# cvlab-kaist/CoPoNeRF

Hardware: AMD Instinct MI355X
Metric: rendered rays/sec (RealEstate10K-shaped 256x256 stereo pair, full-image render, 64 samples/ray) (higher is better)
Workload: dtype f16 (fp16-input/fp32-accumulate MFMA for the per-sample MLPs; f32 decoder; f64 geometry island); 1 GPU; configs[1]: 256x256 stereo pair (narrow rig), full-image render 65536 rays x 64 samples, 1 pair(s) per GPU, render path only (z/rel_pose/flow given, val=True); chunk_rays=65536, lanes=1, pairs_per_gpu=1

## Files before the change

### coponerf_amd/csrc/ufc_conv4d.hip

```cpp
#include <algorithm>
#include <cstdlib>

#include "common.h"
#include "conv4d_geometry.h"

namespace {

__device__ __forceinline__ void gn_publish(double s1, double s2, double* __restrict__ stats, int b) {
    __shared__ int last_flag;
    __shared__ double tree[2][256];
    const unsigned W = gridDim.x * gridDim.y, me = blockIdx.x + gridDim.x * blockIdx.y, B = gridDim.z;
    unsigned long long* part = reinterpret_cast<unsigned long long*>(stats + 3 * (size_t)B + 2 * ((size_t)b * W));
    if (threadIdx.x == 0) {
        const unsigned long long o1 = __hip_atomic_exchange(part + 2 * me, (unsigned long long)__double_as_longlong(s1),
                                                            __ATOMIC_RELAXED, __HIP_MEMORY_SCOPE_AGENT);
        const unsigned long long o2 = __hip_atomic_exchange(part + 2 * me + 1, (unsigned long long)__double_as_longlong(s2),
                                                            __ATOMIC_RELAXED, __HIP_MEMORY_SCOPE_AGENT);
        unsigned zero;
        asm volatile("v_and_b32 %0, 0, %1\n\tv_and_b32 %0, %0, %2" : "=&v"(zero) : "v"((unsigned)o1), "v"((unsigned)o2));
        unsigned long long* cnt = reinterpret_cast<unsigned long long*>(stats + 2 * (size_t)B + b);
        const unsigned long long ticket = __hip_atomic_fetch_add(cnt, 1ULL + zero, __ATOMIC_RELAXED, __HIP_MEMORY_SCOPE_AGENT);
        last_flag = ticket == (unsigned long long)W - 1;
    }
    __syncthreads();
    if (!last_flag) return;
    double a1 = 0.0, a2 = 0.0;
    for (unsigned w = threadIdx.x; w < W; w += 256) {
        a1 += __longlong_as_double((long long)__hip_atomic_load(part + 2 * w, __ATOMIC_RELAXED, __HIP_MEMORY_SCOPE_AGENT));
        a2 += __longlong_as_double((long long)__hip_atomic_load(part + 2 * w + 1, __ATOMIC_RELAXED, __HIP_MEMORY_SCOPE_AGENT));
    }
    tree[0][threadIdx.x] = a1;
    tree[1][threadIdx.x] = a2;
    __syncthreads();
    for (int n = 128; n > 0; n >>= 1) {
        if ((int)threadIdx.x < n) {
            tree[0][threadIdx.x] += tree[0][threadIdx.x + n];
            tree[1][threadIdx.x] += tree[1][threadIdx.x + n];
        }
        __syncthreads();
    }
    if (threadIdx.x == 0) {
        stats[2 * (size_t)b] = tree[0][0];
        stats[2 * (size_t)b + 1] = tree[1][0];
    }
}

__device__ __forceinline__ void gn_publish_block(double s1, double s2, double* __restrict__ stats, int b) {
#pragma unroll
    for (int off = 32; off > 0; off >>= 1) {
        s1 += __shfl_xor(s1, off);
        s2 += __shfl_xor(s2, off);
    }
    __shared__ double red[8];
    const int lane = threadIdx.x & 63, wave = threadIdx.x >> 6;
    if (lane == 0) { red[wave * 2] = s1; red[wave * 2 + 1] = s2; }
    __syncthreads();
    gn_publish(red[0] + red[2] + red[4] + red[6], red[1] + red[3] + red[5] + red[7], stats, b);
}

__global__ __launch_bounds__(256) void conv4d_kernel(const float* __restrict__ x, const float* __restrict__ wq,
                                                     const float* __restrict__ bq, const float* __restrict__ ws,
                                                     const float* __restrict__ bs, int Cin, int Hq, int Wq, int Hs,
                                                     int Ws, int k, int s, int p, int Oq, int Pq_, int Os, int Ps_,
                                                     float* __restrict__ y, double* __restrict__ stats) {
    const int o = blockIdx.y, b = blockIdx.z, Cout = gridDim.y;
    const long long npos = (long long)Oq * Pq_ * Os * Ps_;
    const long long pos = (long long)blockIdx.x * blockDim.x + threadIdx.x;
    float val = 0.0f;
    const bool active = pos < npos;
    if (active) {
        int sx = (int)(pos % Ps_);
        long long t = pos / Ps_;
        const int sy = (int)(t % Os); t /= Os;
        const int qx = (int)(t % Pq_);
        const int qy = (int)(t / Pq_);
        const size_t cstride = (size_t)Hq * Wq * Hs * Ws;
        const float* xb = x + (size_t)b * Cin * cstride;
        float acc = bq[o] + bs[o];
        for (int c = 0; c < Cin; ++c) {
            const float* xc = xb + c * cstride;
            const float* wqc = wq + ((size_t)o * Cin + c) * k * k;
            const float* wsc = ws + ((size_t)o * Cin + c) * k * k;
            for (int i = 0; i < k; ++i)
                for (int j = 0; j < k; ++j) {
                    const int Y = qy * s + i - p, X = qx * s + j - p;
                    if (Y >= 0 && Y < Hq && X >= 0 && X < Wq) {
                        const float* base = xc + ((size_t)Y * Wq + X) * Hs * Ws;
                        float m = -INFINITY;
                        for (int dy = 0; dy < s; ++dy)
                            for (int dx = 0; dx < s; ++dx) {
                                const int yy = sy * s + dy, xx = sx * s + dx;
                                if (yy < Hs && xx < Ws) m = fmaxf(m, base[(size_t)yy * Ws + xx]);
                            }
                        acc += wqc[i * k + j] * m;
                    }
                    const int U = sy * s + i - p, Vv = sx * s + j - p;
                    if (U >= 0 && U < Hs && Vv >= 0 && Vv < Ws) {
                        float m = -INFINITY;
                        for (int dy = 0; dy < s; ++dy)
                            for (int dx = 0; dx < s; ++dx) {
                                const int yy = qy * s + dy, xx = qx * s + dx;
                                if (yy < Hq && xx < Wq) m = fmaxf(m, xc[(((size_t)yy * Wq + xx) * Hs + U) * Ws + Vv]);
                            }
                        acc += wsc[i * k + j] * m;
                    }
                }
        }
        val = acc;
        y[((size_t)b * Cout + o) * npos + pos] = acc;
    }
    double s1 = active ? (double)val : 0.0, s2 = active ? (double)val * val : 0.0;
    gn_publish_block(s1, s2, stats, b);
}

__global__ __launch_bounds__(256) void pool_support_kernel(const float* __restrict__ x, int Hs, int Ws, int s, int Os,
                                                           int Ps_, long long planes, float* __restrict__ out) {
    const long long total = planes * Os * Ps_;
    for (long long i = (long long)blockIdx.x * blockDim.x + threadIdx.x; i < total; i += (long long)gridDim.x * blockDim.x) {
        const int sx = (int)(i % Ps_);
        long long t = i / Ps_;
        const int sy = (int)(t % Os);
        const long long pl = t / Os;
        const float* base = x + pl * Hs * Ws;
        float m = -INFINITY;
        for (int dy = 0; dy < s; ++dy)
            for (int dx = 0; dx < s; ++dx) {
                const int yy = sy * s + dy, xx = sx * s + dx;
                if (yy < Hs && xx < Ws) m = fmaxf(m, base[(size_t)yy * Ws + xx]);
            }
        out[i] = m;
    }
}

__global__ __launch_bounds__(256) void pool_query_kernel(const float* __restrict__ x, int Hq, int Wq, int Hs, int Ws,
                                                         int s, int Oq, int Pq_, long long bc, float* __restrict__ out) {
    const long long P = (long long)Hs * Ws, total = bc * Oq * Pq_ * P;
    for (long long i = (long long)blockIdx.x * blockDim.x + threadIdx.x; i < total; i += (long long)gridDim.x * blockDim.x) {
        const long long uv = i % P;
        long long t = i / P;
        const int qx = (int)(t % Pq_); t /= Pq_;
        const int qy = (int)(t % Oq);
        const long long c = t / Oq;
        const float* base = x + c * Hq * Wq * P + uv;
        float m = -INFINITY;
        for (int dy = 0; dy < s; ++dy)
            for (int dx = 0; dx < s; ++dx) {
                const int yy = qy * s + dy, xx = qx * s + dx;
                if (yy < Hq && xx < Wq) m = fmaxf(m, base[((size_t)yy * Wq + xx) * P]);
            }
        out[i] = m;
    }
}

__global__ __launch_bounds__(256) void conv4d_pooled_kernel(const float* __restrict__ ps, const float* __restrict__ pq,
                                                            const float* __restrict__ wq, const float* __restrict__ bq,
                                                            const float* __restrict__ ws, const float* __restrict__ bs,
                                                            int Cin, int Hq, int Wq, int Hs, int Ws, int k, int s, int p,
                                                            int Oq, int Pq_, int Os, int Ps_, float* __restrict__ y,
                                                            double* __restrict__ stats) {
    const int o = blockIdx.y, b = blockIdx.z, Cout = gridDim.y;
    const long long npos = (long long)Oq * Pq_ * Os * Ps_;
    const long long pos = (long long)blockIdx.x * blockDim.x + threadIdx.x;
    float val = 0.0f;
    const bool active = pos < npos;
    if (active) {
        int sx = (int)(pos % Ps_);
        long long t = pos / Ps_;
        const int sy = (int)(t % Os); t /= Os;
        const int qx = (int)(t % Pq_);
        const int qy = (int)(t / Pq_);
        const size_t ps_c = (size_t)Hq * Wq * Os * Ps_, pq_c = (size_t)Oq * Pq_ * Hs * Ws;
        const float* psb = ps + (size_t)b * Cin * ps_c;
        const float* pqb = pq + (size_t)b * Cin * pq_c;
        float acc = bq[o] + bs[o];
        for (int c = 0; c < Cin; ++c) {
            const float* wqc = wq + ((size_t)o * Cin + c) * k * k;
            const float* wsc = ws + ((size_t)o * Cin + c) * k * k;
            for (int i = 0; i < k; ++i)
                for (int j = 0; j < k; ++j) {
                    const int Y = qy * s + i - p, X = qx * s + j - p;
                    if (Y >= 0 && Y < Hq && X >= 0 && X < Wq)
                        acc += wqc[i * k + j] * psb[c * ps_c + (((size_t)Y * Wq + X) * Os + sy) * Ps_ + sx];
                    const int U = sy * s + i - p, Vv = sx * s + j - p;
                    if (U >= 0 && U < Hs && Vv >= 0 && Vv < Ws)
                        acc += wsc[i * k + j] * pqb[c * pq_c + (((size_t)qy * Pq_ + qx) * Hs + U) * Ws + Vv];
                }
        }
        val = acc;
        y[((size_t)b * Cout + o) * npos + pos] = acc;
    }
    double s1 = active ? (double)val : 0.0, s2 = active ? (double)val * val : 0.0;
    gn_publish_block(s1, s2, stats, b);
}

__global__ __launch_bounds__(256) void conv4d_pooled_c8_kernel(const float* __restrict__ ps, const float* __restrict__ pq,
                                                               const float* __restrict__ wq, const float* __restrict__ bq,
                                                               const float* __restrict__ ws, const float* __restrict__ bs,
                                                               int Cin, int Hq, int Wq, int Hs, int Ws, int k, int s, int p,
                                                               int Oq, int Pq_, int Os, int Ps_, float* __restrict__ y,
                                                               double* __restrict__ stats) {
    extern __shared__ __attribute__((aligned(16))) float wl[];
    const int b = blockIdx.z, kk = k * k;
    for (int i = threadIdx.x; i < Cin * kk * 16; i += 256) {
        const int o = i & 7, br = (i >> 3) & 1, t = i >> 4;
        wl[i] = (br ? ws : wq)[(size_t)o * Cin * kk + t];
    }
    __syncthreads();
    const long long npos = (long long)Oq * Pq_ * Os * Ps_;
    const long long pos = (long long)blockIdx.x * blockDim.x + threadIdx.x;
    const bool active = pos < npos;
    double s1 = 0.0, s2 = 0.0;
    if (active) {
        const int sx = (int)(pos % Ps_);
        long long t = pos / Ps_;
        const int sy = (int)(t % Os); t /= Os;
        const int qx = (int)(t % Pq_);
        const int qy = (int)(t / Pq_);
        const size_t ps_c = (size_t)Hq * Wq * Os * Ps_, pq_c = (size_t)Oq * Pq_ * Hs * Ws;
        const float* psb = ps + (size_t)b * Cin * ps_c;
        const float* pqb = pq + (size_t)b * Cin * pq_c;
        float acc[8];
#pragma unroll
        for (int o = 0; o < 8; ++o) acc[o] = bq[o] + bs[o];
        for (int c = 0; c < Cin; ++c)
            for (int i = 0; i < k; ++i)
                for (int j = 0; j < k; ++j) {
                    const int Y = qy * s + i - p, X = qx * s + j - p;
                    const int U = sy * s + i - p, Vv = sx * s + j - p;
                    const bool okq = Y >= 0 && Y < Hq && X >= 0 && X < Wq, oks = U >= 0 && U < Hs && Vv >= 0 && Vv < Ws;
                    const float vq = okq ? psb[c * ps_c + (((size_t)Y * Wq + X) * Os + sy) * Ps_ + sx] : 0.0f;
                    const float vs = oks ? pqb[c * pq_c + (((size_t)qy * Pq_ + qx) * Hs + U) * Ws + Vv] : 0.0f;
                    const f32x4* w4 = reinterpret_cast<const f32x4*>(wl + (size_t)(c * kk + i * k + j) * 16);
                    const f32x4 a0 = w4[0], a1 = w4[1], b0 = w4[2], b1 = w4[3];
#pragma unroll
                    for (int e = 0; e < 4; ++e) {
                        if (okq) { acc[e] += a0[e] * vq; acc[4 + e] += a1[e] * vq; }
                        if (oks) { acc[e] += b0[e] * vs; acc[4 + e] += b1[e] * vs; }
                    }
                }
#pragma unroll
        for (int o = 0; o < 8; ++o) {
            y[((size_t)b * 8 + o) * npos + pos] = acc[o];
            s1 += (double)acc[o];
            s2 += (double)acc[o] * acc[o];
        }
    }
    gn_publish_block(s1, s2, stats, b);
}

template <int COUT, bool PF, bool DGRAD = false>
__global__ __launch_bounds__(256, PF ? 2 : 4) void conv4d_k3s1_kernel(const float* __restrict__ x, const float* __restrict__ wq,
                                                          const float* __restrict__ bq, const float* __restrict__ ws,
                                                          const float* __restrict__ bs, int Cin, int Hq, int Wq,
                                                          int Hs, int Ws, int cout_total, float* __restrict__ y,
                                                          double* __restrict__ stats) {
    extern __shared__ __attribute__((aligned(16))) float wl[];
    const int b = blockIdx.z;
    const int o0 = blockIdx.y * COUT;
    for (int i = threadIdx.x; i < Cin * 9 * 2 * COUT; i += 256) {
        const int o = o0 + i % COUT;
        int t = i / COUT;
        const int br = t & 1; t >>= 1;
        const int tap = t % 9, c = t / 9;
        wl[i] = DGRAD ? (br ? ws : wq)[((size_t)c * cout_total + o) * 9 + (8 - tap)]
                      : (br ? ws : wq)[((size_t)o * Cin + c) * 9 + tap];
    }
    __syncthreads();
    const long long npos = (long long)Hq * Wq * Hs * Ws;
    const long long pos = (long long)blockIdx.x * blockDim.x + threadIdx.x;
    const bool active = pos < npos;
    double s1 = 0.0, s2 = 0.0;
    if (active) {
        const int sx = (int)(pos % Ws);
        long long t = pos / Ws;
        const int sy = (int)(t % Hs); t /= Hs;
        const int qx = (int)(t % Wq);
        const int qy = (int)(t / Wq);
        float acc[COUT];
#pragma unroll
        for (int o = 0; o < COUT; ++o) acc[o] = DGRAD ? 0.0f : bq[o0 + o] + bs[o0 + o];
        const __amdgpu_buffer_rsrc_t rs = __builtin_amdgcn_make_buffer_rsrc(
            (void*)(x + (size_t)b * Cin * (size_t)npos), 0, (int)((size_t)Cin * npos * 4), 0x00020000);
        int off[18];
#pragma unroll
        for (int i = 0; i < 3; ++i)
#pragma unroll
            for (int j = 0; j < 3; ++j) {
                const int t = i * 3 + j;
                const int Y = qy + i - 1, X = qx + j - 1, U = sy + i - 1, Vv = sx + j - 1;
                const bool okq = Y >= 0 && Y < Hq && X >= 0 && X < Wq, oks = U >= 0 && U < Hs && Vv >= 0 && Vv < Ws;
                off[2 * t] = okq ? (((Y * Wq + X) * Hs + sy) * Ws + sx) * 4 : 0x7ffffff0;
                off[2 * t + 1] = oks ? (((qy * Wq + qx) * Hs + U) * Ws + Vv) * 4 : 0x7ffffff0;
            }
        auto load_taps = [&](int c, float (&xv)[18]) {
            const int cbase = c * (int)npos * 4;
#pragma unroll
            for (int t = 0; t < 18; ++t)
                xv[t] = __builtin_bit_cast(float, __builtin_amdgcn_raw_buffer_load_b32(rs, off[t], cbase, 0));
        };
        auto accumulate = [&](int c, const float (&xv)[18]) {
#pragma unroll
            for (int t = 0; t < 9; ++t) {
                const f32x4* w4 = reinterpret_cast<const f32x4*>(wl + ((c * 9 + t) * 2) * COUT);
                const float vq = xv[2 * t], vs = xv[2 * t + 1];
#pragma unroll
                for (int o4 = 0; o4 < COUT / 4; ++o4) {
                    const f32x4 a = w4[o4], bb = w4[COUT / 4 + o4];
#pragma unroll
                    for (int e = 0; e < 4; ++e)
                        acc[o4 * 4 + e] = __builtin_fmaf(bb[e], vs, __builtin_fmaf(a[e], vq, acc[o4 * 4 + e]));
                    if ((o4 & 1) == 1) __builtin_amdgcn_sched_barrier(0);
                }
            }
        };
        if (PF) {
            float xa[18], xb2[18];
            load_taps(0, xa);
            int c = 0;
#pragma unroll 1
            for (; c + 2 <= Cin; c += 2) {
                load_taps(c + 1, xb2);
                accumulate(c, xa);
                if (c + 2 < Cin) load_taps(c + 2, xa);
                accumulate(c + 1, xb2);
            }
            if (c < Cin) accumulate(c, xa);
        } else {
#pragma unroll 1
            for (int c = 0; c < Cin; ++c) {
                float xv[18];
                load_taps(c, xv);
                accumulate(c, xv);
            }
        }
#pragma unroll
        for (int o = 0; o < COUT; ++o) {
            y[((size_t)b * cout_total + o0 + o) * npos + pos] = acc[o];
            s1 += (double)acc[o];
            s2 += (double)acc[o] * acc[o];
        }
    }
    if (DGRAD) return;
    gn_publish_block(s1, s2, stats, b);
}

__device__ __forceinline__ void gn_block_stats(const double* __restrict__ stats, int b, double n, float eps, float& mean,
                                               float& rstd) {
    __shared__ float mr[2];
    if (threadIdx.x == 0) {
        const double m = stats[2 * (size_t)b] / n;
        const double var = stats[2 * (size_t)b + 1] / n - m * m;
        mr[0] = (float)m;
        mr[1] = (float)(1.0 / sqrt(var + (double)eps));
    }
    __syncthreads();
    mean = mr[0];
    rstd = mr[1];
}

__global__ __launch_bounds__(256) void gn_relu_kernel(const float* y, const double* __restrict__ stats,
                                                      const float* __restrict__ gamma, const float* __restrict__ beta,
                                                      const float* __restrict__ res, float eps, int Cout, long long npos,
                                                      float* out) {
    const int b = blockIdx.z, o = blockIdx.y;
    const long long pos = (long long)blockIdx.x * blockDim.x + threadIdx.x;
    float mean, rstd;
    gn_block_stats(stats, b, (double)Cout * (double)npos, eps, mean, rstd);
    if (pos >= npos) return;
    const size_t idx = ((size_t)b * Cout + o) * npos + pos;
    const float v = (y[idx] - mean) * rstd * gamma[o] + beta[o];
    out[idx] = res ? res[idx] + fmaxf(v, 0.0f) : fmaxf(v, 0.0f);
}

template <int MT, bool DGRAD>
__global__ __launch_bounds__(256, 2) void conv4d_k3s1_mfma_kernel(const float* __restrict__ x, const float* __restrict__ wq,
                                                                  const float* __restrict__ bq, const float* __restrict__ ws,
                                                                  const float* __restrict__ bs, int Cin, int Hq, int Wq, int Hs,
                                                                  int Ws, int cout_total, float* __restrict__ y,
                                                                  double* __restrict__ stats) {
    extern __shared__ __attribute__((aligned(16))) float wl[];
    const int b = blockIdx.z;
    constexpr int CO = MT * 16;
    const int lane = threadIdx.x & 63, wave = threadIdx.x >> 6;
    const int fi = lane & 15, g = lane >> 4;
    const long long npos = (long long)Hq * Wq * Hs * Ws;
    const long long pos = ((long long)blockIdx.x * 4 + wave) * 64 + 4 * fi;
    const bool active = pos < npos;
    const long long pc = active ? pos : 0;
    const int sx = (int)(pc % Ws);
    long long t = pc / Ws;
    const int sy = (int)(t % Hs); t /= Hs;
    const int qx = (int)(t % Wq);
    const int qy = (int)(t / Wq);
    const __amdgpu_buffer_rsrc_t rs = __builtin_amdgcn_make_buffer_rsrc(
        (void*)(x + (size_t)b * Cin * (size_t)npos), 0, (int)((size_t)Cin * npos * 4), 0x00020000);
    const int plane = (int)npos * 4;
    constexpr int kOOB = 0x7ffffff0;
    int offq[9], offs[3];
#pragma unroll
    for (int i = 0; i < 3; ++i) {
#pragma unroll
        for (int j = 0; j < 3; ++j) {
            const int Y = qy + i - 1, X = qx + j - 1;
            const bool ok = active && Y >= 0 && Y < Hq && X >= 0 && X < Wq;
            offq[i * 3 + j] = ok ? (((Y * Wq + X) * Hs + sy) * Ws + sx) * 4 + g * plane : kOOB;
        }
        const int U = sy + i - 1;
        offs[i] = (active && U >= 0 && U < Hs) ? (((qy * Wq + qx) * Hs + U) * Ws + sx) * 4 + g * plane : kOOB;
    }
    const bool row_first = sx == 0, row_last = sx + 4 == Ws;
    f32x4 acc[MT][4];
#pragma unroll
    for (int mt = 0; mt < MT; ++mt)
#pragma unroll
        for (int i = 0; i < 4; ++i) {
            const int co = mt * 16 + g * 4 + i;
            const float bias = (DGRAD || co >= cout_total) ? 0.0f : bq[co] + bs[co];
#pragma unroll
            for (int e = 0; e < 4; ++e) acc[mt][e][i] = bias;
        }
    auto load_group = [&](int c0, f32x4 (&vq)[9], f32x4 (&vs)[3]) {
        const int so = c0 * plane;
#pragma unroll
        for (int k = 0; k < 9; ++k) vq[k] = __builtin_bit_cast(f32x4, __builtin_amdgcn_raw_buffer_load_b128(rs, offq[k], so, 0));
#pragma unroll
        for (int k = 0; k < 3; ++k) vs[k] = __builtin_bit_cast(f32x4, __builtin_amdgcn_raw_buffer_load_b128(rs, offs[k], so, 0));
        __builtin_amdgcn_sched_barrier(0);
    };
    auto step = [&](int c0, int k, const f32x4& v) {
        const float* wrow = wl + ((size_t)k * Cin + c0 + g) * CO + fi;
#pragma unroll
        for (int mt = 0; mt < MT; ++mt) {
            const float a = wrow[mt * 16];
#pragma unroll
            for (int e = 0; e < 4; ++e) acc[mt][e] = __builtin_amdgcn_mfma_f32_16x16x4f32(a, v[e], acc[mt][e], 0, 0, 0);
        }
    };
    auto compute_group = [&](int c0, const f32x4 (&vq)[9], const f32x4 (&vs)[3]) {
#pragma unroll
        for (int i = 0; i < 3; ++i) {
            const f32x4 r = vs[i];
            float left, right;
            const float r3 = r[3], r0 = r[0];
            asm volatile("s_nop 1\n\tv_mov_b32_dpp %0, %2 row_shr:1 row_mask:0xf bank_mask:0xf bound_ctrl:1\n\t"
                         "v_mov_b32_dpp %1, %3 row_shl:1 row_mask:0xf bank_mask:0xf bound_ctrl:1"
                         : "=&v"(left), "=&v"(right) : "v"(r3), "v"(r0));
            const f32x4 rm = {row_first ? 0.0f : left, r[0], r[1], r[2]};
            const f32x4 rp = {r[1], r[2], r[3], row_last ? 0.0f : right};
            step(c0, i * 3 + 0, vq[i * 3 + 0]);
            step(c0, 9 + i * 3 + 0, rm);
            step(c0, i * 3 + 1, vq[i * 3 + 1]);
            step(c0, 9 + i * 3 + 1, r);
            step(c0, i * 3 + 2, vq[i * 3 + 2]);
            step(c0, 9 + i * 3 + 2, rp);
        }
        __builtin_amdgcn_sched_barrier(0);
    };
    f32x4 q0[9], s0[3], q1[9], s1v[3];
    load_group(0, q0, s0);
    if (cout_total < CO)
        for (int i = threadIdx.x; i < 18 * Cin * CO; i += 256)
            if (i % CO >= cout_total) wl[i] = 0.0f;
    {
        const int per_branch = cout_total * Cin * 9, total = 2 * per_branch;
        for (int g0 = threadIdx.x; g0 < total; g0 += 1024) {
            float v[4];
#pragma unroll
            for (int u = 0; u < 4; ++u) {
                const int gi = g0 + 256 * u;
                v[u] = gi < total ? (gi < per_branch ? wq[gi] : ws[gi - per_branch]) : 0.0f;
            }
#pragma unroll
            for (int u = 0; u < 4; ++u) {
                const int gi = g0 + 256 * u;
                if (gi >= total) continue;
                const int br = gi >= per_branch, q = gi - br * per_branch;
                const int tapg = q % 9, mid = (q / 9) % (DGRAD ? cout_total : Cin), top = q / (9 * (DGRAD ? cout_total : Cin));
                const int o = DGRAD ? mid : top, c = DGRAD ? top : mid, tap = DGRAD ? 8 - tapg : tapg;
                wl[((size_t)(br * 9 + tap) * Cin + c) * CO + o] = v[u];
            }
        }
    }
    __syncthreads();
    for (int c0 = 0; c0 < Cin; c0 += 8) {
        if (c0 + 4 < Cin) load_group(c0 + 4, q1, s1v);
        compute_group(c0, q0, s0);
        if (c0 + 4 < Cin) {
            if (c0 + 8 < Cin) load_group(c0 + 8, q0, s0);
            compute_group(c0 + 4, q1, s1v);
        }
    }
    double s1 = 0.0, s2 = 0.0;
    if (active) {
#pragma unroll
        for (int mt = 0; mt < MT; ++mt)
#pragma unroll
            for (int i = 0; i < 4; ++i) {
                const int co = mt * 16 + g * 4 + i;
                if (co < cout_total) {
                    const f32x4 v = {acc[mt][0][i], acc[mt][1][i], acc[mt][2][i], acc[mt][3][i]};
                    *reinterpret_cast<f32x4*>(y + ((size_t)b * cout_total + co) * npos + pos) = v;
#pragma unroll
                    for (int e = 0; e < 4; ++e) {
                        s1 += (double)v[e];
                        s2 += (double)v[e] * v[e];
                    }
                }
            }
    }
    if (DGRAD) return;
#pragma unroll
    for (int o = 32; o > 0; o >>= 1) {
        s1 += __shfl_xor(s1, o);
        s2 += __shfl_xor(s2, o);
    }
    __shared__ double red[8];
    if (lane == 0) { red[wave * 2] = s1; red[wave * 2 + 1] = s2; }
    __syncthreads();
    gn_publish(red[0] + red[2] + red[4] + red[6], red[1] + red[3] + red[5] + red[7], stats, b);
}

__global__ __launch_bounds__(256) void gn_relu_bwd_reduce_kernel(
    const float* __restrict__ y, const float* __restrict__ out, const float* __restrict__ dout,
    const double* __restrict__ stats, const float* __restrict__ gamma, float eps, int B, int Cout, long long npos,
    double* __restrict__ red) {
    const int b = blockIdx.z, o = blockIdx.y;
    float mean, rstd;
    gn_block_stats(stats, b, (double)Cout * (double)npos, eps, mean, rstd);
    const float g = gamma[o];
    double a[4] = {0.0, 0.0, 0.0, 0.0};
    const size_t base = ((size_t)b * Cout + o) * npos;
    if ((npos & 3) == 0) {
        const long long n4 = npos >> 2;
        const f32x4* o4 = reinterpret_cast<const f32x4*>(out + base);
        const f32x4* d4 = reinterpret_cast<const f32x4*>(dout + base);
        const f32x4* y4 = reinterpret_cast<const f32x4*>(y + base);
        for (long long q = (long long)blockIdx.x * blockDim.x + threadIdx.x; q < n4; q += (long long)gridDim.x * blockDim.x) {
            const f32x4 ov = o4[q], dv = d4[q], yv = y4[q];
            float s0 = 0.f, s1 = 0.f;
#pragma unroll
            for (int e = 0; e < 4; ++e) {
                const float dz = ov[e] > 0.0f ? dv[e] : 0.0f;
                s0 += dz;
                s1 += dz * ((yv[e] - mean) * rstd);
            }
            a[0] += (double)(s0 * g);
            a[1] += (double)(s1 * g);
            a[2] += (double)s1;
            a[3] += (double)s0;
        }
    } else {
        for (long long pos = (long long)blockIdx.x * blockDim.x + threadIdx.x; pos < npos;
             pos += (long long)gridDim.x * blockDim.x) {
            const float dz = out[base + pos] > 0.0f ? dout[base + pos] : 0.0f;
            const float yh = (y[base + pos] - mean) * rstd;
            a[0] += (double)(dz * g);
            a[1] += (double)(dz * g * yh);
            a[2] += (double)(dz * yh);
            a[3] += (double)dz;
        }
    }
#pragma unroll
    for (int i = 0; i < 4; ++i)
#pragma unroll
        for (int off = 32; off > 0; off >>= 1) a[i] += __shfl_xor(a[i], off);
    __shared__ double sh[4][4];
    const int lane = threadIdx.x & 63, wave = threadIdx.x >> 6;
    if (lane == 0)
        for (int i = 0; i < 4; ++i) sh[wave][i] = a[i];
    __syncthreads();
    if (threadIdx.x < 4) {
        const double v = sh[0][threadIdx.x] + sh[1][threadIdx.x] + sh[2][threadIdx.x] + sh[3][threadIdx.x];
        double* dst = threadIdx.x < 2 ? red + b * 2 + threadIdx.x : red + 2 * B + o * 2 + (threadIdx.x - 2);
        atomicAdd(dst, v);
    }
}

__global__ __launch_bounds__(256) void gn_relu_bwd_apply_kernel(
    const float* __restrict__ y, const float* __restrict__ out, const float* __restrict__ dout,
    const double* __restrict__ stats, const float* __restrict__ gamma, float eps, int B, int Cout, long long npos,
    const double* __restrict__ red, float* __restrict__ dy, float* __restrict__ dgamma, float* __restrict__ dbeta) {
    const int b = blockIdx.z, o = blockIdx.y;
    const long long pos = (long long)blockIdx.x * blockDim.x + threadIdx.x;
    if (blockIdx.x == 0 && b == 0 && threadIdx.x == 0) {
        dgamma[o] = (float)red[2 * B + o * 2];
        dbeta[o] = (float)red[2 * B + o * 2 + 1];
    }
    const double n = (double)Cout * (double)npos;
    float mean, rstd;
    gn_block_stats(stats, b, n, eps, mean, rstd);
    if (pos >= npos) return;
    const float m1 = (float)(red[b * 2] / n), m2 = (float)(red[b * 2 + 1] / n);
    const size_t idx = ((size_t)b * Cout + o) * npos + pos;
    const float dz = out[idx] > 0.0f ? dout[idx] : 0.0f;
    const float yh = (y[idx] - mean) * rstd;
    dy[idx] = rstd * (dz * gamma[o] - m1 - yh * m2);
}

__global__ __launch_bounds__(256) void transpose_pairs_kernel(const float* __restrict__ x, int P, int Q, float* __restrict__ y) {
    __shared__ float tile[32][33];
    const size_t base = (size_t)blockIdx.z * P * Q;
    const int q0 = blockIdx.x * 32, p0 = blockIdx.y * 32;
    const int tx = threadIdx.x & 31, ty = threadIdx.x >> 5;
#pragma unroll
    for (int i = 0; i < 4; ++i) {
        const int p = p0 + ty + i * 8, q = q0 + tx;
        if (p < P && q < Q) tile[ty + i * 8][tx] = x[base + (size_t)p * Q + q];
    }
    __syncthreads();
#pragma unroll
    for (int i = 0; i < 4; ++i) {
        const int q = q0 + ty + i * 8, p = p0 + tx;
        if (p < P && q < Q) y[base + (size_t)q * P + p] = tile[tx][ty + i * 8];
    }
}

inline size_t conv4d_mfma_lds(int cred, int cprod) { return (size_t)18 * cred * ((cprod + 15) / 16) * 16 * sizeof(float); }

bool conv4d_mfma_ok(int cred, int cprod, int Ws, long long npos, const void* x, const void* y) {
    static const bool off = getenv("CPN_CONV4D_MFMA") && getenv("CPN_CONV4D_MFMA")[0] == '0';
    const bool ws_ok = Ws == 4 || Ws == 8 || Ws == 16 || Ws == 32 || Ws == 64;
    return !off && cred % 4 == 0 && cprod <= 32 && conv4d_mfma_lds(cred, cprod) <= 64 * 1024 && ws_ok &&
           npos % 64 == 0 && (long long)cred * npos * 4 < 0x7ffffff0LL - 4LL * npos * 4 && ((uintptr_t)x % 16) == 0 &&
           ((uintptr_t)y % 16) == 0;
}

template <bool DGRAD>
void launch_conv4d_mfma(hipStream_t st, const float* x, const float* wq, const float* bq, const float* ws, const float* bs, int B,
                        int cred, int cprod, int Hq, int Wq, int Hs, int Ws, float* y, double* stats) {
    const dim3 g2(cpn_cdiv((long long)Hq * Wq * Hs * Ws, 256), 1, B);
    auto* kernel = cprod <= 16 ? conv4d_k3s1_mfma_kernel<1, DGRAD> : conv4d_k3s1_mfma_kernel<2, DGRAD>;
    hipLaunchKernelGGL(kernel, g2, dim3(256), conv4d_mfma_lds(cred, cprod), st, x, wq, bq, ws, bs, cred, Hq, Wq, Hs, Ws, cprod, y,
                       stats);
}

}

extern "C" long long cpn_gn_stats_doubles(int B, int Cout, long long npos) {
    const long long wg = std::max<long long>((long long)cpn_cdiv(npos, 256) * Cout, (long long)cpn_cdiv(npos, 64));
    return 3LL * B + 2LL * B * wg;
}

extern "C" long long cpn_conv4d_scratch(int B, int Cin, int Hq, int Wq, int Hs, int Ws, int s) {
    if (s <= 1) return 0;
    const SGeo g{B, Cin, 0, Hq, Wq, Hs, Ws, 0, s, 0, pooled_size(Hq, s), pooled_size(Wq, s), pooled_size(Hs, s), pooled_size(Ws, s)};
    return g.n_ps() + g.n_pq();
}

extern "C" int cpn_conv4d(const float* x, const float* wq, const float* bq, const float* ws, const float* bs, int B,
                          int Cin, int Cout, int Hq, int Wq, int Hs, int Ws, int k, int s, int p, float* y,
                          double* stats, float* scratch, void* stream) {
    CPN_REQUIRE(x && wq && bq && ws && bs && y && stats, CPN_E_ARG, "cpn_conv4d: null pointer");
    CPN_REQUIRE(B > 0 && B < 65536 && Cin > 0 && Cout > 0 && Cout < 65536 && k > 0 && s > 0 && p >= 0, CPN_E_SHAPE,
                "cpn_conv4d: bad shape");
    SGeo g;
    CPN_REQUIRE(make_geo(B, Cin, Cout, Hq, Wq, Hs, Ws, k, s, p, &g), CPN_E_SHAPE,
                "cpn_conv4d: conv output (%d) and pooled size (%d) of the two branches disagree", g.Oq, pooled_size(Hq, s));
    const int Oq = g.Oq, Pq_ = g.Pq, Os = g.Os, Ps_ = g.Ps;
    const long long npos = g.npos();
    const hipStream_t st = (hipStream_t)stream;
    dim3 grid(cpn_cdiv(npos, 256), Cout, B);
    const size_t wbytes = (size_t)Cin * 9 * 2 * Cout * sizeof(float);
    if (k == 3 && s == 1 && p == 1 && conv4d_mfma_ok(Cin, Cout, Ws, npos, x, y)) {
        launch_conv4d_mfma<false>(st, x, wq, bq, ws, bs, B, Cin, Cout, Hq, Wq, Hs, Ws, y, stats);
    } else if (k == 3 && s == 1 && p == 1 && (Cout == 8 || Cout == 32) && wbytes <= 64 * 1024 &&
        (long long)Cin * npos * 4 < 0x7ffffff0LL) {
        const bool small = (long long)B * npos <= 131072;
        const int per = (Cout == 8 && small) ? 4 : 8;
        dim3 g1(cpn_cdiv(npos, 256), Cout / per, B);
        const size_t wb = wbytes / (Cout / per);
        auto* kernel = per == 4 ? conv4d_k3s1_kernel<4, true> : small ? conv4d_k3s1_kernel<8, true> : conv4d_k3s1_kernel<8, false>;
        hipLaunchKernelGGL(kernel, g1, dim3(256), wb, st, x, wq, bq, ws, bs, Cin, Hq, Wq, Hs, Ws, Cout, y, stats);
    } else if (s > 1 && scratch) {
        float* psv = scratch;
        float* pqv = scratch + (size_t)B * Cin * Hq * Wq * Os * Ps_;
        const long long planes = (long long)B * Cin * Hq * Wq;
        const long long n1 = planes * Os * Ps_, n2 = (long long)B * Cin * Oq * Pq_ * Hs * Ws;
        hipLaunchKernelGGL(pool_support_kernel, dim3((unsigned)std::min<long long>(cpn_cdiv(n1, 256), 65536)), dim3(256), 0,
                           st, x, Hs, Ws, s, Os, Ps_, planes, psv);
        hipLaunchKernelGGL(pool_query_kernel, dim3((unsigned)std::min<long long>(cpn_cdiv(n2, 256), 65536)), dim3(256), 0,
                           st, x, Hq, Wq, Hs, Ws, s, Oq, Pq_, (long long)B * Cin, pqv);
        if (Cout == 8 && (size_t)Cin * k * k * 16 * sizeof(float) <= 48 * 1024)
            hipLaunchKernelGGL(conv4d_pooled_c8_kernel, dim3(cpn_cdiv(npos, 256), 1, B), dim3(256),
                               (size_t)Cin * k * k * 16 * sizeof(float), st, psv, pqv, wq, bq, ws, bs, Cin, Hq, Wq, Hs, Ws, k, s, p,
                               Oq, Pq_, Os, Ps_, y, stats);
        else
            hipLaunchKernelGGL(conv4d_pooled_kernel, grid, dim3(256), 0, st, psv, pqv, wq, bq, ws, bs, Cin, Hq, Wq, Hs, Ws, k, s,
                               p, Oq, Pq_, Os, Ps_, y, stats);
    } else {
        hipLaunchKernelGGL(conv4d_kernel, grid, dim3(256), 0, st, x, wq, bq, ws, bs, Cin, Hq, Wq, Hs, Ws, k, s, p, Oq,
                           Pq_, Os, Ps_, y, stats);
    }
    CPN_LAUNCH_CHECK("cpn_conv4d");
    return 0;
}

extern "C" int cpn_conv4d_dgrad(const float* dy, const float* wq, const float* ws, int B, int Cout, int Cin, int Hq, int Wq,
                                int Hs, int Ws, float* dx, void* stream) {
    CPN_REQUIRE(dy && wq && ws && dx, CPN_E_ARG, "cpn_conv4d_dgrad: null pointer");
    CPN_REQUIRE(B > 0 && B < 65536 && Cin > 0 && Cout > 0 && Hq > 0 && Wq > 0 && Hs > 0 && Ws > 0, CPN_E_SHAPE,
                "cpn_conv4d_dgrad: bad shape");
    const long long npos = (long long)Hq * Wq * Hs * Ws;
    CPN_REQUIRE((Cin % 4) == 0 && (long long)Cout * npos * 4 < 0x7ffffff0LL, CPN_E_SHAPE,
                "cpn_conv4d_dgrad: need Cin %% 4 == 0 and a batch element below 2 GiB (Cin=%d)", Cin);
    if (conv4d_mfma_ok(Cout, Cin, Ws, npos, dy, dx)) {
        launch_conv4d_mfma<true>((hipStream_t)stream, dy, wq, nullptr, ws, nullptr, B, Cout, Cin, Hq, Wq, Hs, Ws, dx, nullptr);
        CPN_LAUNCH_CHECK("cpn_conv4d_dgrad");
        return 0;
    }
    const int per = (Cin % 8) == 0 ? 8 : 4;
    const size_t wb = (size_t)Cout * 9 * 2 * per * sizeof(float);
    CPN_REQUIRE(wb <= 64 * 1024, CPN_E_SHAPE, "cpn_conv4d_dgrad: filter slice exceeds 64 KiB of LDS (Cout=%d)", Cout);
    dim3 g1(cpn_cdiv(npos, 256), Cin / per, B);
    auto* kernel = per == 4 ? conv4d_k3s1_kernel<4, false, true> : conv4d_k3s1_kernel<8, false, true>;
    hipLaunchKernelGGL(kernel, g1, dim3(256), wb, (hipStream_t)stream, dy, wq, (const float*)nullptr, ws, (const float*)nullptr,
                       Cout, Hq, Wq, Hs, Ws, Cin, dx, (double*)nullptr);
    CPN_LAUNCH_CHECK("cpn_conv4d_dgrad");
    return 0;
}

extern "C" int cpn_transpose_pairs(const float* x, int N, int P, int Q, float* y, void* stream) {
    CPN_REQUIRE(x && y, CPN_E_ARG, "cpn_transpose_pairs: null pointer");
    CPN_REQUIRE(N > 0 && N < 65536 && P > 0 && Q > 0, CPN_E_SHAPE, "cpn_transpose_pairs: bad shape (N=%d)", N);
    hipLaunchKernelGGL(transpose_pairs_kernel, dim3(cpn_cdiv(Q, 32), cpn_cdiv(P, 32), N), dim3(256), 0, (hipStream_t)stream, x, P,
                       Q, y);
    CPN_LAUNCH_CHECK("cpn_transpose_pairs");
    return 0;
}

extern "C" int cpn_gn_relu(const float* y, const double* stats, const float* gn_w, const float* gn_b, const float* residual,
                           float eps, int B, int C, long long npos, float* out, void* stream) {
    CPN_REQUIRE(y && stats && gn_w && gn_b && out, CPN_E_ARG, "cpn_gn_relu: null pointer");
    CPN_REQUIRE(B > 0 && B < 65536 && C > 0 && C < 65536 && npos > 0, CPN_E_SHAPE, "cpn_gn_relu: bad shape");
    dim3 grid(cpn_cdiv(npos, 256), C, B);
    hipLaunchKernelGGL(gn_relu_kernel, grid, dim3(256), 0, (hipStream_t)stream, y, stats, gn_w, gn_b, residual, eps, C, npos,
                       out);
    CPN_LAUNCH_CHECK("cpn_gn_relu");
    return 0;
}

extern "C" int cpn_conv4d_gn_relu(const float* x, const float* wq, const float* bq, const float* ws, const float* bs,
                                  const float* gn_w, const float* gn_b, const float* residual, float eps, int B, int Cin,
                                  int Cout, int Hq,
                                  int Wq, int Hs, int Ws, int k, int s, int p, float* y, double* stats, float* scratch,
                                  void* stream) {
    CPN_REQUIRE(gn_w && gn_b, CPN_E_ARG, "cpn_conv4d_gn_relu: null pointer");
    int rc = cpn_conv4d(x, wq, bq, ws, bs, B, Cin, Cout, Hq, Wq, Hs, Ws, k, s, p, y, stats, scratch, stream);
    if (rc) return rc;
    SGeo g;
    make_geo(B, Cin, Cout, Hq, Wq, Hs, Ws, k, s, p, &g);
    return cpn_gn_relu(y, stats, gn_w, gn_b, residual, eps, B, Cout, g.npos(), y, stream);
}

extern "C" int cpn_gn_relu_bwd(const float* y, const float* out, const float* dout, const double* stats,
                               const float* gn_w, float eps, int B, int C, long long npos, double* red, float* dy,
                               float* dgn_w, float* dgn_b, void* stream) {
    CPN_REQUIRE(y && out && dout && stats && gn_w && red && dy && dgn_w && dgn_b, CPN_E_ARG,
                "cpn_gn_relu_bwd: null pointer");
    CPN_REQUIRE(B > 0 && B < 65536 && C > 0 && C < 65536 && npos > 0, CPN_E_SHAPE, "cpn_gn_relu_bwd: bad shape");
    const hipStream_t st = (hipStream_t)stream;
    const unsigned bx = (unsigned)std::min<long long>(cpn_cdiv(npos, 4096), 16);
    hipLaunchKernelGGL(gn_relu_bwd_reduce_kernel, dim3(bx, C, B), dim3(256), 0, st, y, out, dout, stats, gn_w, eps, B, C,
                       npos, red);
    CPN_LAUNCH_CHECK("cpn_gn_relu_bwd(reduce)");
    hipLaunchKernelGGL(gn_relu_bwd_apply_kernel, dim3(cpn_cdiv(npos, 256), C, B), dim3(256), 0, st, y, out, dout, stats,
                       gn_w, eps, B, C, npos, red, dy, dgn_w, dgn_b);
    CPN_LAUNCH_CHECK("cpn_gn_relu_bwd(apply)");
    return 0;
}
```

### coponerf_amd/getz.py

```python
from __future__ import annotations

import math
import os
from typing import Sequence, Tuple

import threading

import torch
import torch.nn as nn
import torch.nn.functional as F

from ._hip import stream_handle as _stream_handle

from .ufc_ops import Linear as _Linear, linear as _linear


class _TrunkBatchNorm(nn.BatchNorm2d):
    _tls = threading.local()

    def forward(self, x):
        if not (self.training and self.track_running_stats) or self.momentum is None:
            return super().forward(x)
        pend = getattr(_TrunkBatchNorm._tls, "pending", None)
        if pend is None:
            return super().forward(x)
        pend.append(self.num_batches_tracked)
        return F.batch_norm(x, self.running_mean, self.running_var, self.weight, self.bias, True, self.momentum, self.eps)

    @staticmethod
    def collect_counters():
        _TrunkBatchNorm._tls.pending = []

    @staticmethod
    def flush_counters():
        pend, _TrunkBatchNorm._tls.pending = getattr(_TrunkBatchNorm._tls, "pending", None), None
        if pend:
            with torch.no_grad():
                torch._foreach_add_(pend, 1)


class TrunkBackward:

    def __init__(self):
        self.enabled = os.environ.get("CPN_TRUNK_BWD_F16", "1") != "0"
        self.target = 4.0
        self.trace = None

    def after_step(self, stepped: bool) -> None:
        self.target = min(4.0, self.target * 2.0) if stepped else max(2.0 ** -4, self.target * 0.25)


class _ScaleSlots:
    _pools = {}

    @classmethod
    def take(cls, dev):
        pool = cls._pools.get(dev)
        if pool is None or pool[1] == 128:
            pool = cls._pools[dev] = [torch.zeros(128, 4, dtype=torch.float32, device=dev), 0]
        pool[1] += 1
        return pool[0][pool[1] - 1]


class _ConvF16BwdFn(torch.autograd.Function):

    @staticmethod
    def forward(ctx, x, w, stride, padding, state: TrunkBackward):
        ctx.save_for_backward(x, w)
        ctx.geo, ctx.state = (int(stride), int(padding)), state
        return F.conv2d(x, w, None, stride, padding)

    @staticmethod
    def backward(ctx, dy):
        from ._hip import call
        x, w = ctx.saved_tensors
        st, pd = ctx.geo
        if not (dy.is_contiguous() or dy.is_contiguous(memory_format=torch.channels_last)):
            dy = dy.contiguous()
        if dy.numel() % 4:
            return tuple(torch.ops.aten.convolution_backward(dy, x, w, None, [st, st], [pd, pd], [1, 1], False, [0, 0], 1,
                                                             [ctx.needs_input_grad[0], ctx.needs_input_grad[1], False])[:2]) + (None,) * 3
        slot = _ScaleSlots.take(dy.device)
        dy16 = torch.empty_like(dy, dtype=torch.float16)
        call("cpn_scale_to_f16", dy.data_ptr(), dy.numel(), float(ctx.state.target), slot.data_ptr(), dy16.data_ptr(),
             slot[1:].data_ptr(), _stream_handle())
        need = [ctx.needs_input_grad[0], ctx.needs_input_grad[1], False]
        dx16, dw16, _ = torch.ops.aten.convolution_backward(dy16, x.half(), w.half(), None, [st, st], [pd, pd], [1, 1], False,
                                                            [0, 0], 1, need)
        if ctx.state.trace is not None:
            ctx.state.trace.append((tuple(x.shape), dx16.abs().max() if need[0] else None, dw16.abs().max() if need[1] else None))
        inv = slot[2:3]
        dw = None
        if need[1]:
            dw = torch.empty(w.shape, dtype=torch.float32, device=w.device)
            torch.mul(dw16, inv, out=dw)
        return (dx16 * inv if need[0] else None), dw, None, None, None


def _conv(conv: nn.Conv2d, x, state: TrunkBackward):
    if (state.enabled and x.is_cuda and x.dtype == torch.float32 and torch.is_grad_enabled() and conv.bias is None
            and x.numel() % 4 == 0 and (x.is_contiguous() or x.is_contiguous(memory_format=torch.channels_last))):
        return _ConvF16BwdFn.apply(x, conv.weight, conv.stride[0], conv.padding[0], state)
    return conv(x)


class _BasicBlock(nn.Module):
    def __init__(self, cin: int, cout: int, stride: int, trunk_bwd: TrunkBackward):
        super().__init__()
        self.trunk_bwd = trunk_bwd
        self.conv1 = nn.Conv2d(cin, cout, 3, stride, 1, bias=False)
        self.bn1 = _TrunkBatchNorm(cout)
        self.relu = nn.ReLU(inplace=True)
        self.conv2 = nn.Conv2d(cout, cout, 3, 1, 1, bias=False)
        self.bn2 = _TrunkBatchNorm(cout)
        self.downsample = None
        if stride != 1 or cin != cout:
            self.downsample = nn.Sequential(nn.Conv2d(cin, cout, 1, stride, bias=False), _TrunkBatchNorm(cout))

    def forward(self, x):
        st = self.trunk_bwd
        idt = x if self.downsample is None else self.downsample[1](_conv(self.downsample[0], x, st))
        out = self.bn2(_conv(self.conv2, self.relu(self.bn1(_conv(self.conv1, x, st))), st))
        return self.relu(out + idt)


class _ResNet34Trunk(nn.Module):
    def __init__(self, trunk_bwd: TrunkBackward):
        super().__init__()
        self.conv1 = nn.Conv2d(3, 64, 7, 2, 3, bias=False)
        self.bn1 = _TrunkBatchNorm(64)
        self.relu = nn.ReLU(inplace=True)
        self.maxpool = nn.MaxPool2d(3, 2, 1)
        cin = 64
        for i, (cout, n, s) in enumerate([(64, 3, 1), (128, 4, 2), (256, 6, 2), (512, 3, 2)], start=1):
            setattr(self, f"layer{i}", nn.Sequential(*[_BasicBlock(cin if j == 0 else cout, cout, s if j == 0 else 1, trunk_bwd)
                                                       for j in range(n)]))
            cin = cout
        self.avgpool = nn.Sequential()
        self.fc = nn.Sequential()


def _bn_act(x, bn, relu: bool, res=None):
    from ._hip import call
    N, C, H, W = x.shape
    if not x.is_contiguous() or (H * W) % 4 or (res is not None and not res.is_contiguous()):
        y = F.batch_norm(x, bn.running_mean, bn.running_var, bn.weight, bn.bias, False, 0.0, bn.eps)
        y = y if res is None else y + res
        return F.relu(y) if relu else y
    call("cpn_bn_act", x.data_ptr(), 0 if res is None else res.data_ptr(), bn.running_mean.data_ptr(), bn.running_var.data_ptr(),
         bn.weight.data_ptr(), bn.bias.data_ptr(), float(bn.eps), N, C, H * W, int(relu), x.data_ptr(),
         _stream_handle())
    return x


def _trunk_conv(xh, conv, bn, relu: bool, res=None, want_nchw: bool = False):
    from ._hip import call, lib
    N, H, W, Cin = xh.shape
    Cout, k, s = conv.out_channels, conv.kernel_size[0], conv.stride[0]
    w = conv.weight
    pack = conv.__dict__.get("_cpn_pack")
    if pack is None or pack[0] != (w._version, w.data_ptr()):
        wp = torch.empty(k * k, Cin, Cout, dtype=torch.float32, device=xh.device)
        call("cpn_pack_conv_weight", w.detach().contiguous().data_ptr(), Cout, Cin, k, wp.data_ptr(),
             _stream_handle())
        pack = conv.__dict__["_cpn_pack"] = ((w._version, w.data_ptr()), wp)
    Ho, Wo = (H + 2 * (k // 2) - k) // s + 1, (W + 2 * (k // 2) - k) // s + 1
    out = torch.empty(N, Ho, Wo, Cout, dtype=torch.float32, device=xh.device)
    nchw = torch.empty(N, Cout, Ho, Wo, dtype=torch.float32, device=xh.device) if want_nchw else None
    scratch = torch.empty(lib().cpn_trunk_conv_scratch_floats(N, H, W, Cin, Cout, k, s), dtype=torch.float32, device=xh.device)
    call("cpn_trunk_conv_bn_act", xh.data_ptr(), pack[1].data_ptr(), N, H, W, Cin, Cout, k, s, bn.running_mean.data_ptr(),
         bn.running_var.data_ptr(), bn.weight.data_ptr(), bn.bias.data_ptr(), float(bn.eps),
         0 if res is None else res.data_ptr(), int(relu), out.data_ptr(), 0 if nchw is None else nchw.data_ptr(),
         scratch.data_ptr(), _stream_handle())
    return out, nchw


class SpatialEncoder(nn.Module):

    def __init__(self):
        super().__init__()
        self.trunk_bwd = TrunkBackward()
        self.model = _ResNet34Trunk(self.trunk_bwd)

    def _forward_infer(self, x):
        m = self.model
        x = _bn_act(m.conv1(x), m.bn1, True)
        lat = [x]
        xh = None
        for name in ("layer1", "layer2", "layer3", "layer4"):
            blocks = list(getattr(m, name))
            own = (HIP_TRUNK_TAIL and name in ("layer3", "layer4")
                   and x.shape[0] * (x.shape[2] // 2) * (x.shape[3] // 2) <= HIP_TRUNK_MAX_POSITIONS)
            if own and xh is None:
                xh = x.permute(0, 2, 3, 1).contiguous()
            for i, blk in enumerate(blocks):
                if own:
                    idt = xh
                    if blk.downsample is not None:
                        idt, _ = _trunk_conv(xh, blk.downsample[0], blk.downsample[1], False)
                    out, _ = _trunk_conv(xh, blk.conv1, blk.bn1, True)
                    xh, xn = _trunk_conv(out, blk.conv2, blk.bn2, True, res=idt, want_nchw=i == len(blocks) - 1)
                    x = xn if xn is not None else x
                    continue
                xh = None
                idt = x
                if blk.downsample is not None:
                    idt = _bn_act(blk.downsample[0](x), blk.downsample[1], False)
                out = _bn_act(blk.conv1(x), blk.bn1, True)
                x = _bn_act(blk.conv2(out), blk.bn2, True, res=idt)
            lat.append(x)
        return lat[::-1]

    def forward(self, x):
        m = self.model
        if (not torch.is_grad_enabled() and not self.training and x.is_cuda and x.dtype == torch.float32
                and x.is_contiguous() and FUSED_TRUNK):
            return self._forward_infer(x)
        _TrunkBatchNorm.collect_counters()
        try:
            x = m.relu(m.bn1(m.conv1(x)))
            lat = [x]
            for name in ("layer1", "layer2", "layer3", "layer4"):
                x = getattr(m, name)(x)
                lat.append(x)
        finally:
            _TrunkBatchNorm.flush_counters()
        return lat[::-1]


class Conv4d(nn.Module):

    def __init__(self, cin: int, cout: int, k: int, s: int, p: int):
        super().__init__()
        self.query_conv = nn.Conv2d(cin, cout, (k, k), stride=(s, s), padding=(p, p))
        self.supp_conv = nn.Conv2d(cin, cout, (k, k), stride=(s, s), padding=(p, p))
        self.k, self.s, self.p = k, s, p


class Encoder4D(nn.Module):

    def __init__(self, levels: Sequence[int], k: int = 3, s: int = 1, p: int = 1):
        super().__init__()
        self.conv4d = nn.ModuleList([
            nn.Sequential(Conv4d(levels[i], levels[i + 1], k, s, p), nn.GroupNorm(1, levels[i + 1]), nn.ReLU())
            for i in range(len(levels) - 1)])

    def forward(self, x, ops, residual=None):
        last = len(self.conv4d) - 1
        for i, blk in enumerate(self.conv4d):
            c4, gn = blk[0], blk[1]
            args = (x, c4.query_conv.weight, c4.query_conv.bias, c4.supp_conv.weight, c4.supp_conv.bias, c4.k, c4.s, c4.p,
                    gn.weight, gn.bias, gn.eps)
            x = ops.conv4d_gn_relu(*args, residual=residual) if (i == last and residual is not None) else ops.conv4d_gn_relu(*args)
        return x


class _DWConv(nn.Module):
    def __init__(self, dim: int, size: int):
        super().__init__()
        self.dwconv = nn.Conv2d(dim, dim, 3, 1, 1, bias=True, groups=dim)
        self.size = size

    def forward(self, x):
        B, L, C = x.shape
        if x.is_cuda and x.dtype == torch.float32 and C % 4 == 0:
            from .ufc_ops import DwConvTokensFn
            return DwConvTokensFn.apply(x, self.dwconv.weight, self.dwconv.bias, self.size)
        xm = x.transpose(1, 2).reshape(B, C, self.size, self.size)
        y = self.dwconv(xm)
        return y.flatten(2).transpose(1, 2)


TWO_STREAMS = os.environ.get("CPN_GETZ_TWO_STREAMS", "1") != "0"
BATCH_VIEWS = os.environ.get("CPN_GETZ_BATCH_VIEWS", "1") != "0"
FUSED_TRUNK = os.environ.get("CPN_GETZ_FUSED_TRUNK", "1") != "0"
HIP_TRUNK_TAIL = os.environ.get("CPN_GETZ_HIP_TRUNK_TAIL", "1") != "0"
FUSED_POSE_ENDS = os.environ.get("CPN_GETZ_FUSED_POSE_ENDS", "1") != "0"
HIP_TRUNK_MAX_POSITIONS = int(os.environ.get("CPN_GETZ_HIP_TRUNK_MAX_POSITIONS", "2048"))
CORR_MEAN3_TRAIN = os.environ.get("CPN_CORR_MEAN3_TRAIN", "1") != "0"
_SIDE_STREAMS = {}


def _side_stream(device):
    st = _SIDE_STREAMS.get(device)
    if st is None:
        st = _SIDE_STREAMS[device] = torch.cuda.Stream(device=device)
    return st


def _tokens_to_map(x, h):
    B, L, C = x.shape
    return x.transpose(1, 2).reshape(B, C, h, L // h)


def _map_to_tokens(x):
    return x.flatten(2).transpose(1, 2)


def _corr_to_maps(corr):
    B, H, Hs, Ws, Ht, Wt = corr.shape
    from .ufc_ops import swap_pairs
    return swap_pairs(corr).reshape(B, H * Ht * Wt, Hs, Ws)


class UFCLayer(nn.Module):

    def __init__(self, fs: int, f2c: Tuple[int, int, int], nhead: int = 8, d: int = 256):
        super().__init__()
        self.fs, self.nhead, self.dim = fs, nhead, d // nhead
        self.q_proj = _Linear(d + 256 * nhead, d)
        self.k_proj = _Linear(d + 256 * nhead, d)
        self.v_proj = _Linear(d, d)
        self.v_proj_corr = Encoder4D((nhead, nhead))
        self.mlp = nn.Sequential(_Linear(d, 4 * d), _DWConv(4 * d, fs), nn.GELU(), _Linear(4 * d, d))
        self.mlp_corr = Encoder4D((nhead, 4 * nhead, nhead))
        self.mlp_cross = nn.Sequential(_Linear(d, 4 * d), _DWConv(4 * d, fs), nn.GELU(), _Linear(4 * d, d))
        self.mlp_refine_corr = Encoder4D((nhead, 4 * nhead, nhead))
        self.mlp_refine_corr2 = Encoder4D((nhead, 4 * nhead, nhead))
        self.feat_to_corr1 = Encoder4D((1, nhead), *f2c)
        self.feat_to_corr2 = Encoder4D((1, nhead), *f2c)
        self.norm1, self.norm2 = nn.LayerNorm(d), nn.LayerNorm(d)
        self.v_cross = _Linear(d, d)
        self.norm_cross1, self.norm_cross2 = nn.LayerNorm(d), nn.LayerNorm(d)
        self.pos_embed = nn.Parameter(torch.zeros(1, fs * fs, 1, self.dim))
        nn.init.trunc_normal_(self.pos_embed, std=.02)

    def _feed_forward(self, seq, x):
        if torch.is_grad_enabled() or not x.is_cuda or x.dtype != torch.float32:
            return seq(x)
        from ._hip import call
        h = seq[0](x)
        B, L, C = h.shape
        dw = seq[1]
        if C % 4 or not h.is_contiguous():
            return seq[3](seq[2](dw(h)))
        y = torch.empty_like(h)
        call("cpn_dwconv3x3_tokens", h.data_ptr(), dw.dwconv.weight.detach().reshape(C, 9).data_ptr(),
             dw.dwconv.bias.detach().data_ptr(), B, dw.size, dw.size, C, 2, y.data_ptr(),
             _stream_handle())
        return seq[3](y)

    def _qk_weights(self, ncc: int):
        ps = (self.q_proj.weight, self.k_proj.weight, self.q_proj.bias, self.k_proj.bias, self.pos_embed)
        grad = torch.is_grad_enabled() and any(p.requires_grad for p in ps)
        key = tuple((p.data_ptr(), p._version) for p in ps) + (ncc,)
        c = self.__dict__.get("_qk_cache")
        if not grad and c is not None and c[0] == key:
            return c[1]
        Wq, Wk = ps[0], ps[1]
        (Wq_c, Wq_f), (Wk_c, Wk_f) = Wq.split((ncc, Wq.shape[1] - ncc), 1), Wk.split((ncc, Wk.shape[1] - ncc), 1)
        out = (torch.cat((Wq_c, Wk_c), 0), torch.cat((Wq_f, Wk_f), 0), torch.cat((ps[2], ps[3]), 0),
               self.pos_embed.reshape(-1, self.dim))
        if not grad:
            out = tuple(t.detach().contiguous() for t in out)
            self.__dict__["_qk_cache"] = (key, out)
        return out

    def _queries_keys(self, corr, feat_n, ops):
        B, H, Hs, Ws, Ht, Wt = corr.shape
        fs, d = self.fs, self.nhead * self.dim
        Wc, Wf, bqk, pos = self._qk_weights(H * Ht * Wt)
        low = torch.matmul(Wc, _corr_to_maps(corr).flatten(2)).view(B, 2 * d, Hs, Ws)
        lin = _linear(feat_n, Wf, bqk)
        if torch.is_grad_enabled() and (lin.requires_grad or low.requires_grad) or not lin.is_cuda:
            qk = (lin + _map_to_tokens(ops.resize_bilinear(low, fs))).view(B, -1, 2, self.nhead, self.dim) + pos[None, :, None, None, :]
            return qk.unbind(2)
        from ._hip import call
        q = torch.empty(B, fs * fs, self.nhead, self.dim, dtype=torch.float32, device=lin.device)
        k = torch.empty_like(q)
        call("cpn_qk_assemble", lin.data_ptr(), low.data_ptr(), pos.data_ptr(), B, fs, Hs, Ws, self.nhead, self.dim,
             q.data_ptr(), k.data_ptr(), _stream_handle())
        return q, k

    def _attention(self, corr, feat, ops):
        B, H, Hs, Ws, Ht, Wt = corr.shape
        fs = self.fs
        feat_r = feat
        feat = self.norm1(feat)
        q, k = self._queries_keys(corr, feat, ops)
        vf = self.v_proj(feat).view(B, -1, self.nhead, self.dim)
        msg_feat = ops.linear_attention(q, k, vf).view(B, -1, self.nhead * self.dim)
        msg_corr = ops.cost_volume_attention(q, k, self.v_proj_corr(corr, ops), fs, residual=corr)
        msg_feat = feat_r + msg_feat
        msg_feat = msg_feat + self._feed_forward(self.mlp, self.norm2(msg_feat))
        msg_corr = self.mlp_corr(msg_corr, ops, residual=msg_corr)
        return msg_corr, msg_feat

    def _cross(self, corr, src, trg, ops):
        B, H, Hs, Ws, Ht, Wt = corr.shape
        fs = self.fs
        c = corr.reshape(B, H, Hs * Ws, Ht * Wt)
        pool = lambda t, hh: _map_to_tokens(F.avg_pool2d(_tokens_to_map(t, fs), fs // hh))
        trg_v = self.v_cross(self.norm_cross1(pool(trg, Ht))).view(B, -1, self.nhead, self.dim)
        src_v = self.v_cross(self.norm_cross1(pool(src, Hs))).view(B, -1, self.nhead, self.dim)
        src_attn, trg_attn = ops.cross_attention(c, src_v, trg_v)
        src_attn = src_attn.reshape(B, -1, self.nhead * self.dim)
        trg_attn = trg_attn.reshape(B, -1, self.nhead * self.dim)
        up = lambda t, hh: _map_to_tokens(_tokens_to_map(t, hh).repeat_interleave(fs // hh, 2)
                                          .repeat_interleave(fs // hh, 3))
        src = src + up(src_attn, Hs)
        trg = trg + up(trg_attn, Ht)
        src = src + self._feed_forward(self.mlp_cross, self.norm_cross2(src))
        trg = trg + self._feed_forward(self.mlp_cross, self.norm_cross2(trg))
        return src, trg

    def _cross_views(self, corr, x2, ops):
        B, H, Hs, Ws, Ht, Wt = corr.shape
        fs, d = self.fs, self.nhead * self.dim
        c = corr.reshape(B, H, Hs * Ws, Ht * Wt)
        pooled = _map_to_tokens(F.avg_pool2d(_tokens_to_map(x2, fs), fs // Hs))
        v = self.v_cross(self.norm_cross1(pooled)).view(2 * B, -1, self.nhead, self.dim)
        v_src, v_trg = v.chunk(2, 0)
        src_attn, trg_attn = ops.cross_attention(c, v_src, v_trg)
        attn = torch.cat((src_attn.reshape(B, -1, d), trg_attn.reshape(B, -1, d)), 0)
        r = fs // Hs
        x2 = x2 + _map_to_tokens(_tokens_to_map(attn, Hs).repeat_interleave(r, 2).repeat_interleave(r, 3))
        return x2 + self._feed_forward(self.mlp_cross, self.norm_cross2(x2))

    def _forward_views_batched(self, corr, src, trg, ops):
        t4 = lambda x: x.permute(0, 1, 4, 5, 2, 3)
        from .ufc_ops import swap_pairs as _swap
        B = corr.shape[0]
        corr2 = torch.cat((corr, _swap(corr)), 0)
        msg2, x2 = self._attention(corr2, torch.cat((src, trg), 0), ops)
        msg_s, msg_t = msg2.chunk(2, 0)
        xs, xt = x2.chunk(2, 0)
        corr_r = msg_s + t4(msg_t)
        corr_r = self.feat_to_corr1(ops.correlation_tokens(xs, xt, self.fs), ops, residual=corr_r)
        corr_r = self.mlp_refine_corr(corr_r, ops, residual=corr_r)
        x2 = self._cross_views(corr_r, x2, ops)
        xs, xt = x2.chunk(2, 0)
        corr_r = self.feat_to_corr2(ops.correlation_tokens(xs, xt, self.fs), ops, residual=corr_r)
        corr_r = self.mlp_refine_corr2(corr_r, ops, residual=corr_r)
        return corr_r, xs, xt

    def forward(self, corr, src, trg, ops):
        if BATCH_VIEWS and corr.shape[2:4] == corr.shape[4:6] and src.shape == trg.shape:
            return self._forward_views_batched(corr, src, trg, ops)
        t4 = lambda x: x.permute(0, 1, 4, 5, 2, 3)
        from .ufc_ops import swap_pairs as _swap
        if corr.is_cuda and TWO_STREAMS and torch.cuda.is_current_stream_capturing():
            cur = torch.cuda.current_stream()
            side = _side_stream(corr.device)
            side.wait_stream(cur)
            with torch.cuda.stream(side):
                corr_trg, trg_r = self._attention(_swap(corr), trg, ops)
            corr_src, src_r = self._attention(corr, src, ops)
            cur.wait_stream(side)
            corr_trg.record_stream(cur)
            trg_r.record_stream(cur)
        else:
            corr_src, src_r = self._attention(corr, src, ops)
            corr_trg, trg_r = self._attention(_swap(corr), trg, ops)
        corr_r = corr_src + t4(corr_trg)
        corr_r = self.feat_to_corr1(ops.correlation_tokens(src_r, trg_r, self.fs), ops, residual=corr_r)
        corr_r = self.mlp_refine_corr(corr_r, ops, residual=corr_r)
        src_r, trg_r = self._cross(corr_r, src_r, trg_r, ops)
        corr_r = self.feat_to_corr2(ops.correlation_tokens(src_r, trg_r, self.fs), ops, residual=corr_r)
        corr_r = self.mlp_refine_corr2(corr_r, ops, residual=corr_r)
        return corr_r, src_r, trg_r


def _interp_tokens(x, size, ops):
    h = int(math.isqrt(x.shape[1]))
    return _map_to_tokens(ops.resize_bilinear(_tokens_to_map(x, h), size))


def _interp4d(x, n, ops):
    B, C, Hs, Ws, Ht, Wt = x.shape
    if Hs == n and Ht == n:
        return x
    y = ops.resize_bilinear(x.reshape(B, C * Hs * Ws, Ht, Wt), n)
    y = y.reshape(B, C, Hs, Ws, n, n).permute(0, 1, 4, 5, 2, 3).reshape(B, C * n * n, Hs, Ws)
    y = ops.resize_bilinear(y, n)
    return y.reshape(B, C, n, n, n, n).permute(0, 1, 4, 5, 2, 3)


_GRID_CONSTS = {}


def _mapping_to_flow(m):
    B, _, H, W = m.shape
    key = (H, W, str(m.device))
    c = _GRID_CONSTS.get(key)
    if c is None:
        xs = torch.arange(W, device=m.device, dtype=torch.float32).view(1, 1, 1, W).expand(1, 1, H, W)
        ys = torch.arange(H, device=m.device, dtype=torch.float32).view(1, 1, H, 1).expand(1, 1, H, W)
        c = _GRID_CONSTS[key] = (torch.cat((xs, ys), 1).contiguous(),
                                 torch.tensor([(W - 1) / 2.0, (H - 1) / 2.0], device=m.device).view(1, 2, 1, 1))
    grid, half = c
    return (m[:, :2].float() + 1) * half - grid


class UFC(nn.Module):

    def __init__(self, nhead: int = 8):
        super().__init__()
        cfg = [(16, (3, 1, 1), 2), (32, (3, 2, 1), 2), (64, (5, 4, 2), 1)]
        self.layers = nn.ModuleList([nn.ModuleList([UFCLayer(fs, f2c, nhead) for _ in range(n)]) for fs, f2c, n in cfg])
        self.embedding = nn.ModuleList([Encoder4D((1, nhead), *f2c) for _, f2c, _ in cfg])
        self.proj_feat = nn.ModuleList([nn.Sequential(_Linear(c, 256), nn.ReLU()) for c in (512, 256, 128)])

    def forward(self, feat: Sequence[torch.Tensor], nview: int, ops):
        B2 = feat[0].shape[0]
        B = B2 // nview
        proj = [self.proj_feat[i](_map_to_tokens(feat[i])) for i in range(3)]
        proj = [p.view(B, nview, *p.shape[1:]) for p in proj]
        src_f = [p[:, 0] for p in proj]
        trg_f = [p[:, 1] for p in proj]
        feats, corrs = [], []
        corr = src = trg = None
        for lvl, fs in enumerate((16, 32, 64)):
            emb = self.embedding[lvl](ops.correlation_tokens(src_f[lvl], trg_f[lvl], fs), ops, residual=corr)
            if lvl == 0:
                corr, src, trg = emb, src_f[0], trg_f[0]
            else:
                corr = emb
                src = _interp_tokens(src, fs, ops) + src_f[lvl]
                trg = _interp_tokens(trg, fs, ops) + trg_f[lvl]
            for layer in self.layers[lvl]:
                corr, src, trg = layer(corr, src, trg, ops)
            feats.append(_tokens_to_map(torch.stack((src, trg), dim=1).flatten(0, 1), fs))
            corrs.append(ops.correlation_tokens(src, trg, fs))
        fused_ok = CORR_MEAN3_TRAIN or not (torch.is_grad_enabled() and corrs[2].requires_grad)
        if len(corrs) == 3 and hasattr(ops, "corr_mean3") and corrs[2].shape[-1] == 64 and fused_ok:
            c = ops.corr_mean3(corrs)
        else:
            up = [_interp4d(x, 64, ops) for x in corrs]
            c = ((up[0] + up[1]) + up[2]) / len(corrs)
        t_to_s, s_to_t = ops.soft_argmax_pair(c)
        return feats, (_mapping_to_flow(t_to_s), _mapping_to_flow(s_to_t), t_to_s, s_to_t), c


def positional_encodings(fx, fy, cx, cy, n: int = 64):
    B = fx.shape[0]
    dev = fx.device
    hp, wp = cy * 2, cx * 2
    a = (fx / wp) * 2
    b = (fy / hp) * 2
    c = (cx / wp) * 2 - 1
    d = (cy / hp) * 2 - 1
    key = ("pe", n, str(dev))
    g = _GRID_CONSTS.get(key)
    if g is None:
        lin = torch.linspace(-1, 1, steps=n, device=dev)
        g = _GRID_CONSTS[key] = (lin.repeat_interleave(n)[None].contiguous(), lin.repeat(n)[None].contiguous(),
                                 torch.ones(1, n * n, device=dev))
    xs, ys, ones = g
    p4 = (xs - c) / a
    p3 = (ys - d) / b
    return torch.stack((p3 * p3, p4 * p4, p3 * p4, p3, p4, ones.expand(B, -1)), dim=2)


class _Mlp(nn.Module):
    def __init__(self, d: int, hidden: int):
        super().__init__()
        self.fc1, self.act, self.fc2 = _Linear(d, hidden), nn.GELU(), _Linear(hidden, d)

    def forward(self, x):
        return self.fc2(self.act(self.fc1(x)))


class _CrossAttention(nn.Module):
    def __init__(self, dim: int):
        super().__init__()
        self.qkv = _Linear(dim, dim * 3, bias=False)
        self.proj_fundamental = _Linear(dim + 6, dim)

    def forward(self, x1, x2, corr, intr, ops):
        B = x1.shape[0]
        a1 = corr.reshape(B, corr.shape[-4] * corr.shape[-3], -1)
        f1 = ops.dual_softmax(a1)
        f2 = f1.transpose(-2, -1)
        n = int(math.isqrt(x1.shape[1]))
        if isinstance(intr[0], str):
            pos = ops.pose_positional(intr[1], intr[2], n).to(x1.dtype)
        else:
            pos = positional_encodings(*intr, n=n).to(x1.dtype)
        v1, v2 = torch.cat([x1, pos], dim=2), torch.cat([x2, pos], dim=2)
        F1 = ((v1.transpose(-2, -1) @ f1) @ v1).transpose(-2, -1)
        F2 = ((v2.transpose(-2, -1) @ f2) @ v2).transpose(-2, -1)
        return self.proj_fundamental(F2), self.proj_fundamental(F1)


class CrossBlock(nn.Module):
    def __init__(self, dim: int = 256):
        super().__init__()
        self.norm1 = nn.LayerNorm(dim)
        self.cross_attn = _CrossAttention(dim)
        self.norm2 = nn.LayerNorm(dim)
        self.mlp = _Mlp(dim, 4 * dim)
        self.norm = nn.LayerNorm(dim)

    def forward(self, x, corr, intr, ops):
        b_s, hw, nf = x.shape
        x = x.reshape(-1, 2, hw, nf)
        fa, fb = self.cross_attn(self.norm1(x[:, 0]), self.norm1(x[:, 1]), corr, intr, ops)
        f = torch.cat([fa.unsqueeze(1), fb.unsqueeze(1)], dim=1).reshape(b_s, -1, nf)
        f = f + self.mlp(self.norm2(f))
        return self.norm(f)


def r6d_to_matrix(d6):
    a1, a2 = d6[..., :3], d6[..., 3:]
    b1 = F.normalize(a1, dim=-1)
    b2 = F.normalize(a2 - (b1 * a2).sum(-1, keepdim=True) * b1, dim=-1)
    return torch.stack((b1, b2, torch.cross(b1, b2, dim=-1)), dim=-2)


_CONSTS = {}


def _const(device, values):
    key = (str(device), tuple(values))
    if key not in _CONSTS:
        _CONSTS[key] = torch.tensor(values, dtype=torch.float32, device=device)
    return _CONSTS[key]


def imagenet_normalise(x):
    mean = _const(x.device, (0.485, 0.456, 0.406)).view(1, 3, 1, 1)
    std = _const(x.device, (0.229, 0.224, 0.225)).view(1, 3, 1, 1)
    return (x - mean) / std


def make_pose_heads():
    mlp = lambda dims: [m for i in range(len(dims) - 1) for m in (nn.ReLU(), _Linear(dims[i], dims[i + 1]))]
    pose = nn.Sequential(_Linear((16 * 16 + 6) * 256 * 2, 512), nn.ReLU(), _Linear(512, 256), nn.ReLU(),
                         _Linear(256, 128 * 2), nn.ReLU())
    return pose, nn.Sequential(*mlp([128, 64, 32, 6])), nn.Sequential(*mlp([128, 64, 32, 3]))


_DET_OWNED = [False]


def _conv_determinism(want: bool) -> None:
    cd = torch.backends.cudnn
    if want and not cd.deterministic:
        cd.deterministic = True
        _DET_OWNED[0] = True
    elif not want and _DET_OWNED[0] and cd.deterministic:
        cd.deterministic = False
        _DET_OWNED[0] = False


def get_z(model, input, ops):
    rgb = input["context"]["rgb"]
    B, V, H, W, _ = rgb.shape
    if (H, W) != (256, 256):
        raise ValueError("get_z supports 256x256 context images only, like the reference (SURVEY.md §0)")
    model.H, model.W = H, W
    x = imagenet_normalise((rgb.flatten(0, 1).permute(0, 3, 1, 2) + 1) / 2.)
    det = not torch.is_grad_enabled() and getattr(model, "deterministic_get_z", True)
    _conv_determinism(det)
    z = model.encoder(x.contiguous() if det else x)[:3]
    infer = not torch.is_grad_enabled()
    z_conv, z_conv_nhwc16 = ops.conv_map(rgb.flatten(0, 1), model.conv_map.weight, model.conv_map.bias, want_nhwc16=infer)
    if z_conv_nhwc16 is not None and hasattr(model, "_engine"):
        model._engine.adopt_level3(z_conv, z_conv_nhwc16)
    feats, flows, c = model.feature_cost_aggregation(z, model.n_view, ops)
    fused_pose = infer and FUSED_POSE_ENDS and hasattr(ops, "pose_tail") and rgb.is_cuda
    if fused_pose:
        intr = ("raw", input["context"]["intrinsics"], H)
    else:
        Kn = input["context"]["intrinsics"].clone()
        Kn[:, :, :2, :] = Kn[:, :, :2, :] / H
        intr = (Kn[:, 0, 0, 0, None], Kn[:, 0, 1, 1, None], Kn[:, 0, 0, 2, None], Kn[:, 0, 1, 2, None])
    pose_feat = model.cross_attention(feats[-1].flatten(-2, -1).transpose(-1, -2), c, intr, ops).reshape(B, -1)
    if fused_pose:
        rel_pose = ops.pose_tail(pose_feat, model.pose_regressor, model.rotation_regressor, model.translation_regressor)
        return feats + [z_conv], rel_pose, flows
    lat = model.pose_regressor(pose_feat)[:, :128]
    R = r6d_to_matrix(model.rotation_regressor(lat))[:, :3, :3]
    t = model.translation_regressor(lat)
    bottom = _const(t.device, (0., 0., 0., 1.)).expand(B, 1, -1)
    rel_pose = torch.cat((torch.cat((R, t.unsqueeze(-1)), dim=-1), bottom), dim=1)
    return feats + [z_conv], rel_pose, flows
```

### coponerf_amd/ufc_ops.py

```python
from __future__ import annotations

import os

import torch
import torch.nn.functional as F
from torch.autograd import Function

from . import _hip
from ._hip import call


def _stream() -> int:
    return _hip.stream_handle()


class _HipForwardVjp(Function):

    @staticmethod
    def forward(ctx, hip_fn, vjp_fn, *tensors):
        out = hip_fn(*tensors)
        ctx.vjp_fn = vjp_fn
        ctx.save_for_backward(*tensors)
        return out

    @staticmethod
    def backward(ctx, *gouts):
        need = ctx.needs_input_grad[2:]
        with torch.enable_grad():
            ins = [t.detach().requires_grad_(n) for t, n in zip(ctx.saved_tensors, need)]
            outs = ctx.vjp_fn(*ins)
            outs = outs if isinstance(outs, tuple) else (outs,)
            wanted = [t for t, n in zip(ins, need) if n]
            pairs = [(o, g) for o, g in zip(outs, gouts) if g is not None]
            got = torch.autograd.grad([o for o, _ in pairs], wanted, [g for _, g in pairs], allow_unused=True)
        it = iter(got)
        return (None, None) + tuple(next(it) if n else None for n in need)


WGRAD_MIN_ROWS = 256


def wgrad_f32(dY2, X2, want_bias: bool):
    R, O = dY2.shape
    I = X2.shape[1]
    ok = (dY2.is_cuda and dY2.dtype == torch.float32 and X2.dtype == torch.float32
          and (R >= WGRAD_MIN_ROWS or O * I >= (1 << 24)) and O % 4 == 0 and I % 4 == 0)
    if ok:
        if dY2.stride(1) != 1 or dY2.stride(0) % 4 or dY2.stride(0) < O or dY2.data_ptr() % 16:
            dY2 = dY2.contiguous()
        if X2.stride(1) != 1 or X2.stride(0) % 4 or X2.stride(0) < I or X2.data_ptr() % 16:
            X2 = X2.contiguous()
        dW = torch.empty(O, I, dtype=torch.float32, device=dY2.device)
        db = torch.empty(O, dtype=torch.float32, device=dY2.device) if want_bias else None
        scratch = torch.empty(_hip.lib().cpn_wgrad_f32_scratch_floats(R, O, I), dtype=torch.float32, device=dY2.device)
        call("cpn_wgrad_f32", dY2.data_ptr(), dY2.stride(0), X2.data_ptr(), X2.stride(0), R, O, I, dW.data_ptr(),
             0 if db is None else db.data_ptr(), scratch.data_ptr(), _stream())
        return dW, db
    return dY2.t() @ X2, (dY2.sum(0) if want_bias else None)


class LinearFn(Function):

    @staticmethod
    def forward(ctx, x, weight, bias):
        ctx.save_for_backward(x, weight)
        ctx.has_bias = bias is not None
        if (x.dim() == 2 and x.shape[0] <= 4 and x.shape[1] >= (1 << 15) and x.shape[1] % 4 == 0 and x.is_contiguous()
                and weight.is_contiguous() and x.data_ptr() % 16 == 0 and weight.data_ptr() % 16 == 0):
            nsplit, O = 8, weight.shape[0]
            h = torch.empty(x.shape[0], O, nsplit, dtype=torch.float32, device=x.device)
            call("cpn_pose_gemv", x.data_ptr(), weight.data_ptr(), x.shape[0], x.shape[1], O, nsplit, h.data_ptr(), _stream())
            y = h.sum(-1)
            return y if bias is None else y + bias
        return F.linear(x, weight, bias)

    @staticmethod
    def backward(ctx, dy):
        x, w = ctx.saved_tensors
        if not dy.is_contiguous():
            dy = dy.contiguous()
        dx = dy.matmul(w) if ctx.needs_input_grad[0] else None
        dW = db = None
        if ctx.needs_input_grad[1] or (ctx.has_bias and ctx.needs_input_grad[2]):
            dW, db = wgrad_f32(dy.reshape(-1, dy.shape[-1]), x.reshape(-1, x.shape[-1]),
                               ctx.has_bias and ctx.needs_input_grad[2])
        return dx, dW, db


def linear(x, weight, bias=None):
    if (x.is_cuda and x.dtype == torch.float32 and torch.is_grad_enabled()
            and (x.numel() // x.shape[-1] >= WGRAD_MIN_ROWS or weight.numel() >= (1 << 24))
            and (weight.requires_grad or (bias is not None and bias.requires_grad))):
        return LinearFn.apply(x, weight, bias)
    return F.linear(x, weight, bias)


class Linear(torch.nn.Linear):

    def forward(self, x):
        return linear(x, self.weight, self.bias)


class _CorrelationFn(Function):

    @staticmethod
    def forward(ctx, ops, src, trg, fs):
        out, sn, tn = ops._correlation(src, trg, fs)
        ctx.save_for_backward(src, trg, sn, tn)
        return out

    @staticmethod
    def backward(ctx, gout):
        src, trg, sn, tn = ctx.saved_tensors
        B, L, _ = src.shape
        dC = gout.reshape(B, L, L)

        def through_norm(x, xn, dxn):
            if x.is_cuda and x.shape[-1] <= 1024:
                x_, xn_, d_ = x.contiguous().float(), xn.contiguous(), dxn.contiguous()
                dx = torch.empty_like(d_)
                call("cpn_l2norm_rows_bwd", x_.data_ptr(), xn_.data_ptr(), d_.data_ptr(), x_.numel() // x_.shape[-1], x_.shape[-1],
                     1e-5, dx.data_ptr(), _stream())
                return dx
            r = x.norm(dim=-1, p=2, keepdim=True)
            return dxn / (r + 1e-5) - xn * ((xn * dxn).sum(-1, keepdim=True) / r.clamp_min(1e-30))

        ds = through_norm(src, sn, torch.bmm(dC, tn)) if ctx.needs_input_grad[1] else None
        dt = through_norm(trg, tn, torch.bmm(dC.transpose(1, 2), sn)) if ctx.needs_input_grad[2] else None
        return None, ds, dt, None


def _linear_attention_splits(L):
    return max(1, min(64, L // 64))


class _LinearAttentionFn(Function):

    @staticmethod
    def forward(ctx, ops, q, k, v, channel_major, eps):
        q, k, v = q.contiguous(), k.contiguous(), v.contiguous()
        ctx.save_for_backward(q, k, v)
        ctx.cm, ctx.eps = channel_major, eps
        with torch.no_grad():
            return ops.linear_attention(q, k, v, channel_major, eps)

    @staticmethod
    def backward(ctx, gout):
        q, k, v = ctx.saved_tensors
        B, L, H, _ = q.shape
        Dv = v.shape[2] if ctx.cm else v.shape[3]
        nsplit = _linear_attention_splits(L)
        g = gout.contiguous().float()
        scr = torch.empty(_hip.lib().cpn_linear_attention_bwd_scratch(B, L, H, Dv, nsplit), dtype=torch.float32, device=q.device)
        dq, dk, dv = torch.empty_like(q), torch.empty_like(k), torch.empty_like(v)
        call("cpn_linear_attention_bwd", q.data_ptr(), k.data_ptr(), v.data_ptr(), g.data_ptr(), B, L, H, Dv, int(ctx.cm),
             float(ctx.eps), nsplit, scr.data_ptr(), dq.data_ptr(), dk.data_ptr(), dv.data_ptr(), _stream())
        return None, dq, dk, dv, None, None


class _CrossAttentionFn(Function):

    @staticmethod
    def forward(ctx, ops, c, src_v, trg_v):
        c, src_v, trg_v = c.contiguous(), src_v.contiguous(), trg_v.contiguous()
        with torch.no_grad():
            sa, ta = ops.cross_attention(c, src_v, trg_v)
        ctx.save_for_backward(c, src_v, trg_v, sa, ta)
        return sa, ta

    @staticmethod
    def backward(ctx, g1, g2):
        c, sv, tv, sa, ta = ctx.saved_tensors
        B, H, S, T = c.shape
        g1 = torch.zeros_like(sa) if g1 is None else g1.contiguous().float()
        g2 = torch.zeros_like(ta) if g2 is None else g2.contiguous().float()
        scr = torch.empty(_hip.lib().cpn_cross_attention_bwd_scratch(B, H, S, T), dtype=torch.float32, device=c.device)
        dc, dsv, dtv = torch.empty_like(c), torch.empty_like(sv), torch.empty_like(tv)
        call("cpn_cross_attention_bwd", c.data_ptr(), sv.data_ptr(), tv.data_ptr(), sa.data_ptr(), ta.data_ptr(), g1.data_ptr(),
             g2.data_ptr(), B, H, S, T, sv.shape[-1], scr.data_ptr(), dc.data_ptr(), dsv.data_ptr(), dtv.data_ptr(), _stream())
        return None, dc, dsv, dtv


STRIDED_HIP_VJP = os.environ.get("CPN_STRIDED_CONV4D_VJP", "1") != "0"


def _wants_grad(*tensors) -> bool:
    return torch.is_grad_enabled() and any(t.requires_grad for t in tensors)


def _pool_pair(x, s, support: bool):
    if s == 1:
        return x
    B, C, Hq, Wq, Hs, Ws = x.shape
    if support:
        y = F.max_pool2d(x.reshape(B * C * Hq * Wq, 1, Hs, Ws), s, s, 0, ceil_mode=True)
        return y.reshape(B, C, Hq, Wq, y.shape[-2], y.shape[-1])
    y = F.max_pool2d(x.permute(0, 1, 4, 5, 2, 3).reshape(B * C * Hs * Ws, 1, Hq, Wq), s, s, 0, ceil_mode=True)
    return y.reshape(B, C, Hs, Ws, y.shape[-2], y.shape[-1]).permute(0, 1, 4, 5, 2, 3)


def _conv4d_lib(x, wq, bq, ws, bs, s, p):
    B, Cin = x.shape[:2]
    xq, xs = _pool_pair(x, s, True), _pool_pair(x, s, False)
    Hq, Wq, Hs2, Ws2 = xq.shape[2:]
    yq = F.conv2d(xq.permute(0, 4, 5, 1, 2, 3).reshape(B * Hs2 * Ws2, Cin, Hq, Wq), wq, bq, stride=s, padding=p)
    yq = yq.reshape(B, Hs2, Ws2, -1, yq.shape[-2], yq.shape[-1]).permute(0, 3, 4, 5, 1, 2)
    Hq2, Wq2, Hs, Ws = xs.shape[2:]
    ys = F.conv2d(xs.permute(0, 2, 3, 1, 4, 5).reshape(B * Hq2 * Wq2, Cin, Hs, Ws), ws, bs, stride=s, padding=p)
    ys = ys.reshape(B, Hq2, Wq2, -1, ys.shape[-2], ys.shape[-1]).permute(0, 3, 1, 2, 4, 5)
    return yq + ys


class _Conv4dGnReluFn(Function):

    @staticmethod
    def forward(ctx, ops, x, wq, bq, ws, bs, gn_w, gn_b, k, s, p, eps):
        y, out, stats = ops._conv4d_gn_relu_hip(x, wq, bq, ws, bs, k, s, p, gn_w, gn_b, eps, keep_pre=True)
        ctx.save_for_backward(x, wq, bq, ws, bs, gn_w, y, out, stats)
        ctx.cfg = (k, s, p, eps)
        ctx.ops = ops
        return out

    @staticmethod
    def backward(ctx, dout):
        x, wq, bq, ws, bs, gn_w, y, out, stats = ctx.saved_tensors
        k, s, p, eps = ctx.cfg
        B, C = y.shape[:2]
        npos = y[0, 0].numel()
        dev = y.device
        dout = dout.contiguous().float()
        red = ctx.ops._zeros64(B * 2 + C * 2, dev)
        dy = torch.empty_like(y)
        dgw = torch.empty(C, dtype=torch.float32, device=dev)
        dgb = torch.empty(C, dtype=torch.float32, device=dev)
        gw = gn_w.detach().contiguous().float()
        call("cpn_gn_relu_bwd", y.data_ptr(), out.data_ptr(), dout.data_ptr(), stats.data_ptr(), gw.data_ptr(), float(eps),
             B, C, npos, red.data_ptr(), dy.data_ptr(), dgw.data_ptr(), dgb.data_ptr(), _stream())
        need_x, need_w = ctx.needs_input_grad[1], any(ctx.needs_input_grad[2:6])
        gx = gwq = gbq = gws = gbs = None
        if k == 3 and s == 1 and p == 1:
            Bx, Cin, Hq, Wq, Hs, Ws = x.shape
            if need_x and Cin % 4 == 0:
                gx = torch.empty_like(x)
                fw = lambda w: w.detach().contiguous().float()
                wq_c, ws_c = fw(wq), fw(ws)
                call("cpn_conv4d_dgrad", dy.data_ptr(), wq_c.data_ptr(), ws_c.data_ptr(), B, C, Cin, Hq, Wq, Hs, Ws,
                     gx.data_ptr(), _stream())
            elif need_x:
                flip = lambda w: w.detach().float().flip(-1, -2).transpose(0, 1).contiguous()
                zb = torch.zeros(Cin, dtype=torch.float32, device=dev)
                gx = torch.empty_like(x)
                scratch = torch.zeros(int(_hip.lib().cpn_gn_stats_doubles(B, Cin, Hq * Wq * Hs * Ws)), dtype=torch.float64,
                                      device=dev)
                wq_t, ws_t = flip(wq), flip(ws)
                call("cpn_conv4d", dy.data_ptr(), wq_t.data_ptr(), zb.data_ptr(), ws_t.data_ptr(), zb.data_ptr(), B, C, Cin,
                     Hq, Wq, Hs, Ws, 3, 1, 1, gx.data_ptr(), scratch.data_ptr(), 0, _stream())
            if need_w and Cin <= 32 and C <= 32 and Hs * Ws <= 256 and Hq * Wq <= 256 and min(Ws, Wq) >= 4:
                gwq = torch.empty(C, Cin, 3, 3, dtype=torch.float32, device=dev)
                gws = torch.empty(C, Cin, 3, 3, dtype=torch.float32, device=dev)
                gbs = torch.empty(C, dtype=torch.float32, device=dev)
                part = torch.empty(_hip.lib().cpn_conv_wgrad_scratch(Cin, C), dtype=torch.float32, device=dev)
                xf = x.detach().contiguous().float()
                call("cpn_conv_wgrad_planes", xf.data_ptr(), dy.data_ptr(), B, Cin, C, Hq * Wq, Hs, Ws, part.data_ptr(),
                     gws.data_ptr(), gbs.data_ptr(), _stream())
                xt = _swap_pairs_hip(xf)
                dt = _swap_pairs_hip(dy)
                call("cpn_conv_wgrad_planes", xt.data_ptr(), dt.data_ptr(), B, Cin, C, Hs * Ws, Hq, Wq, part.data_ptr(),
                     gwq.data_ptr(), 0, _stream())
                gbq = gbs
            elif need_w:
                cb = torch.ops.aten.convolution_backward
                xq = x.permute(0, 4, 5, 1, 2, 3).reshape(B * Hs * Ws, Cin, Hq, Wq)
                dq = dy.permute(0, 4, 5, 1, 2, 3).reshape(B * Hs * Ws, C, Hq, Wq)
                _, gwq, gbq = cb(dq, xq, wq.detach(), [C], [1, 1], [1, 1], [1, 1], False, [0, 0], 1, [False, True, True])
                xs = x.permute(0, 2, 3, 1, 4, 5).reshape(B * Hq * Wq, Cin, Hs, Ws)
                ds = dy.permute(0, 2, 3, 1, 4, 5).reshape(B * Hq * Wq, C, Hs, Ws)
                _, gws, _ = cb(ds, xs, ws.detach(), [C], [1, 1], [1, 1], [1, 1], False, [0, 0], 1, [False, True, False])
                gbs = gbq
        elif (s > 1 and STRIDED_HIP_VJP and x.is_cuda and C == 8 and x.shape[1] in (1, 2, 8) and k <= 7 and (need_x or need_w)
              and x.numel() < 2 ** 31):
            Bx, Cin, Hq, Wq, Hs, Ws = x.shape
            xf = x.detach().contiguous().float()
            fw = lambda w: w.detach().contiguous().float()
            scr = torch.empty(int(_hip.lib().cpn_conv4d_strided_bwd_scratch(Bx, Cin, C, Hq, Wq, Hs, Ws, k, s, p)),
                              dtype=torch.float32, device=dev)
            if need_x:
                gx = torch.empty_like(xf)
            if need_w:
                gwq = torch.empty(C, Cin, k, k, dtype=torch.float32, device=dev)
                gws = torch.empty_like(gwq)
                gbq = gbs = torch.empty(C, dtype=torch.float32, device=dev)
            ptr = lambda t: 0 if t is None else t.data_ptr()
            call("cpn_conv4d_strided_bwd", xf.data_ptr(), dy.data_ptr(), fw(wq).data_ptr(), fw(ws).data_ptr(), Bx, Cin, C, Hq, Wq,
                 Hs, Ws, k, s, p, scr.data_ptr(), ptr(gx), ptr(gwq), ptr(gws), ptr(gbq), _stream())
        else:
            need = ctx.needs_input_grad[1:6]
            with torch.enable_grad():
                ins = [t.detach().requires_grad_(n) for t, n in zip((x, wq, bq, ws, bs), need)]
                yy = _conv4d_lib(*ins, s, p)
            wanted = [t for t, n in zip(ins, need) if n]
            got = iter(torch.autograd.grad(yy, wanted, dy) if wanted else ())
            gx, gwq, gbq, gws, gbs = (next(got) if n else None for n in need)
        return None, gx, gwq, gbq, gws, gbs, dgw, dgb, None, None, None, None


class _DualSoftmaxFn(Function):

    @staticmethod
    def forward(ctx, a):
        a = a.contiguous().float()
        B, L, M = a.shape
        dev = a.device
        rstat = torch.empty(B, L, 2, dtype=torch.float32, device=dev)
        cstat = torch.empty(B, M, 2, dtype=torch.float32, device=dev)
        f = torch.empty_like(a)
        call("cpn_dual_softmax", a.data_ptr(), B, L, M, rstat.data_ptr(), cstat.data_ptr(), f.data_ptr(), _stream())
        ctx.save_for_backward(a, rstat, cstat, f)
        return f

    @staticmethod
    def backward(ctx, df):
        a, rstat, cstat, f = ctx.saved_tensors
        B, L, M = a.shape
        df = df.contiguous().float()
        srow = torch.empty(B, L, dtype=torch.float32, device=a.device)
        scol = torch.empty(B, M, dtype=torch.float32, device=a.device)
        da = torch.empty_like(a)
        call("cpn_dual_softmax_bwd", a.data_ptr(), rstat.data_ptr(), cstat.data_ptr(), f.data_ptr(), df.data_ptr(), B, L, M,
             srow.data_ptr(), scol.data_ptr(), da.data_ptr(), _stream())
        return da


class _SoftArgmaxPairFn(Function):

    @staticmethod
    def forward(ctx, ops, c):
        t_to_s, s_to_t = ops._soft_argmax_pair_hip(c)
        ctx.save_for_backward(c, t_to_s, s_to_t)
        return t_to_s, s_to_t

    @staticmethod
    def backward(ctx, g_ts, g_st):
        c, t_to_s, s_to_t = ctx.saved_tensors
        B, h = c.shape[0], c.shape[-1]
        zero = lambda g, like: torch.zeros_like(like) if g is None else g.contiguous().float()
        g_ts, g_st = zero(g_ts, t_to_s), zero(g_st, s_to_t)
        dc = torch.empty_like(c)
        call("cpn_soft_argmax_pair_bwd", c.data_ptr(), B, h, 0.02, t_to_s.data_ptr(), s_to_t.data_ptr(), g_ts.data_ptr(),
             g_st.data_ptr(), dc.data_ptr(), _stream())
        return None, dc


class DwConv3x3Fn(Function):

    @staticmethod
    def forward(ctx, x, w, b):
        ctx.save_for_backward(x, w)
        ctx.has_b = b is not None
        return F.conv2d(x, w, b, 1, 1, 1, x.shape[1])

    @staticmethod
    def backward(ctx, dy):
        x, w = ctx.saved_tensors
        N, C, H, W = x.shape
        dy = dy.contiguous().float()
        dx = F.conv2d(dy, w.detach().flip(-1, -2), None, 1, 1, 1, C) if ctx.needs_input_grad[0] else None
        dw = db = None
        if ctx.needs_input_grad[1] or ctx.needs_input_grad[2]:
            xf = x.detach().contiguous().float()
            dw = torch.empty(C, 1, 3, 3, dtype=torch.float32, device=x.device)
            db = torch.empty(C, dtype=torch.float32, device=x.device) if ctx.has_b else None
            call("cpn_dwconv3x3_wgrad", xf.data_ptr(), dy.data_ptr(), N, C, H, W, dw.data_ptr(),
                 0 if db is None else db.data_ptr(), _stream())
        return dx, dw, db


def _swap_pairs_hip(x):
    xc = x.contiguous().float()
    B, C, a, b, c, d = xc.shape
    y = torch.empty(B, C, c, d, a, b, dtype=torch.float32, device=xc.device)
    if B * C >= 65536:
        return xc.permute(0, 1, 4, 5, 2, 3).contiguous()
    call("cpn_transpose_pairs", xc.data_ptr(), B * C, a * b, c * d, y.data_ptr(), _stream())
    return y


class SwapPairsFn(Function):

    @staticmethod
    def forward(ctx, x):
        return _swap_pairs_hip(x)

    @staticmethod
    def backward(ctx, dy):
        return _swap_pairs_hip(dy)


def swap_pairs(x):
    if x.is_cuda and x.dim() == 6:
        return SwapPairsFn.apply(x) if torch.is_grad_enabled() and x.requires_grad else _swap_pairs_hip(x)
    return x.permute(0, 1, 4, 5, 2, 3).contiguous()


class DwConvTokensFn(Function):

    @staticmethod
    def forward(ctx, x, w, b, size: int):
        B, L, C = x.shape
        xc = x.detach().contiguous().float()
        wc = w.detach().reshape(C, 9).contiguous().float()
        bc = None if b is None else b.detach().contiguous().float()
        y = torch.empty_like(xc)
        call("cpn_dwconv3x3_tokens", xc.data_ptr(), wc.data_ptr(), 0 if bc is None else bc.data_ptr(), B, size, size, C, 0,
             y.data_ptr(), _stream())
        ctx.save_for_backward(xc, wc)
        ctx.size, ctx.has_b, ctx.wshape = size, b is not None, tuple(w.shape)
        return y

    @staticmethod
    def backward(ctx, dy):
        xc, wc = ctx.saved_tensors
        B, L, C = xc.shape
        dyc = dy.contiguous().float()
        dx = dw = db = None
        if ctx.needs_input_grad[0]:
            dx = torch.empty_like(xc)
            call("cpn_dwconv3x3_tokens", dyc.data_ptr(), wc.data_ptr(), 0, B, ctx.size, ctx.size, C, 1, dx.data_ptr(), _stream())
        if ctx.needs_input_grad[1] or ctx.needs_input_grad[2]:
            dw = torch.empty(C, 9, dtype=torch.float32, device=xc.device)
            db = torch.empty(C, dtype=torch.float32, device=xc.device) if ctx.has_b else None
            part = torch.empty(_hip.lib().cpn_dwconv3x3_tokens_wgrad_scratch(B, ctx.size, C), dtype=torch.float32,
                               device=xc.device)
            call("cpn_dwconv3x3_tokens_wgrad", xc.data_ptr(), dyc.data_ptr(), B, ctx.size, ctx.size, C, part.data_ptr(),
                 dw.data_ptr(), 0 if db is None else db.data_ptr(), _stream())
            dw = dw.view(ctx.wshape)
        return dx, dw, db, None


def _resize_adjoint_hip(g, h: int):
    g = g.contiguous().float()
    N, C, H, W = g.shape
    out = torch.empty(N, C, h, h, dtype=torch.float32, device=g.device)
    call("cpn_resize_bilinear_ac_adjoint", g.data_ptr(), out.data_ptr(), N * C, h, h, H, W, _stream())
    return out


class _ResizeFn(Function):

    @staticmethod
    def forward(ctx, ops, x, size):
        ctx.in_shape, ctx.size = tuple(x.shape), size
        return ops.resize_bilinear(x, size)

    @staticmethod
    def backward(ctx, dout):
        if ctx.in_shape[-1] == ctx.in_shape[-2]:
            return None, _resize_adjoint_hip(dout, ctx.in_shape[-1]), None
        return None, torch.ops.aten.upsample_bilinear2d_backward(dout.contiguous(), [ctx.size, ctx.size],
                                                                 list(ctx.in_shape), True, None, None), None


class _CorrMean3Fn(Function):

    @staticmethod
    def forward(ctx, ops, c0, c1, c2):
        ctx.hs = (c0.shape[-1], c1.shape[-1])
        return ops._corr_mean3_hip((c0, c1, c2))

    @staticmethod
    def backward(ctx, g):
        g = g.contiguous().float()
        B, n = g.shape[0], g.shape[-1]
        third = 1.0 / 3.0
        grads = []
        for need, h in zip(ctx.needs_input_grad[1:3], ctx.hs):
            if not need:
                grads.append(None)
                continue
            t = _resize_adjoint_hip(g.view(B, n * n, n, n), h)
            t = t.view(B, n, n, h * h).permute(0, 3, 1, 2)
            t = _resize_adjoint_hip(t, h)
            grads.append((t.view(B, h, h, h, h).permute(0, 3, 4, 1, 2) * third).reshape(B, 1, h, h, h, h))
        g2 = g * third if ctx.needs_input_grad[3] else None
        return None, grads[0], grads[1], g2


class _ResizeAdjointFn(Function):

    @staticmethod
    def forward(ctx, ops, x, size):
        ctx.ops, ctx.n = ops, x.shape[-1]
        return _resize_adjoint_hip(x, size)

    @staticmethod
    def backward(ctx, g):
        return None, ctx.ops.resize_bilinear(g, ctx.n), None


def cost_volume_attention_torch(ops, q, k, v_corr, fs, residual=None, eps=1e-6):
    import torch.nn.functional as F_
    B, H, Hs, Ws, Ht, Wt = v_corr.shape
    D = q.shape[-1]
    Q, K = F_.elu(q) + 1, F_.elu(k) + 1
    Z = 1.0 / (torch.einsum("blhd,bhd->blh", Q, K.sum(dim=1)) + eps)
    as_map = lambda t: t.permute(0, 2, 3, 1).reshape(B, H * D, fs, fs)
    if fs == Hs:
        Qd, Kd = as_map(Q * Z[..., None]), as_map(K)
    else:
        Qd = ops.resize_bilinear(as_map(Q * Z[..., None]), Hs)
        Kd = ops.resize_bilinear_adjoint(as_map(K), Hs)
    Qd, Kd = Qd.reshape(B, H, D, Hs * Ws), Kd.reshape(B, H, D, Hs * Ws)
    M = torch.matmul(Kd, v_corr.reshape(B, H, Hs * Ws, Ht * Wt))
    msg = torch.matmul(Qd.transpose(-1, -2), M).reshape(B, H, Hs, Ws, Ht, Wt)
    return msg if residual is None else residual + msg


def cost_volume_attention_reference_order(ops, q, k, v_corr, fs, residual=None, eps=1e-6):
    B, H, Hs, Ws, Ht, Wt = v_corr.shape
    vc = ops.resize_bilinear(swap_pairs(v_corr).reshape(B, H * Ht * Wt, Hs, Ws), fs)
    msg = ops.linear_attention(q, k, vc.reshape(B, H, Ht * Wt, fs * fs), channel_major=True, eps=eps)
    msg = ops.resize_bilinear(msg.reshape(B, H * Ht * Wt, fs, fs), Hs)
    msg = msg.reshape(B, H, Ht, Wt, Hs, Ws).permute(0, 1, 4, 5, 2, 3)
    return msg if residual is None else residual + msg


_NORM_CONSTS = {}


def _conv_map_lib(rgb, w, b):
    x = (rgb.permute(0, 3, 1, 2) + 1) / 2.
    c = _NORM_CONSTS.get(x.device)
    if c is None:
        c = _NORM_CONSTS[x.device] = (torch.tensor((0.485, 0.456, 0.406), device=x.device).view(1, 3, 1, 1),
                                      torch.tensor((0.229, 0.224, 0.225), device=x.device).view(1, 3, 1, 1))
    mean, std = c
    return F.conv2d((x - mean) / std, w, b, stride=1, padding=3)


_LINSPACE = {}


class HipOps:

    @staticmethod
    def _need_gpu(t):
        if t.device.type != "cuda":
            raise RuntimeError("coponerf_amd UFC operators run on a HIP device only (tensor on %s)" % t.device)

    def _stats(self, B, Cout, npos, device):
        n = int(_hip.lib().cpn_gn_stats_doubles(B, Cout, npos))
        pool = getattr(self, "_stats_pool", None)
        if pool is None or pool[0].device != device or pool[1] + n > pool[0].numel():
            pool = [torch.zeros(max(n, 1 << 20), device=device, dtype=torch.float64), 0]
            self._stats_pool = pool
        i = pool[1]
        pool[1] = i + n + (n & 1)
        return pool[0][i:i + n]

    def _zeros64(self, n, device):
        pool = getattr(self, "_z64_pool", None)
        if pool is None or pool[0].device != device or pool[1] + n > pool[0].numel():
            pool = [torch.zeros(max(8192, n), device=device, dtype=torch.float64), 0]
            self._z64_pool = pool
        i = pool[1]
        pool[1] = i + ((n + 1) // 2) * 2
        return pool[0][i:i + n]

    def conv4d_gn_relu(self, x, wq, bq, ws, bs, k, s, p, gn_w, gn_b, eps, residual=None):
        self._need_gpu(x)
        if _wants_grad(x, wq, bq, ws, bs, gn_w, gn_b) or (residual is not None and _wants_grad(residual)):
            y = _Conv4dGnReluFn.apply(self, x.float(), wq, bq, ws, bs, gn_w, gn_b, k, s, p, eps)
            return y if residual is None else residual + y
        if residual is not None and not (residual.is_contiguous() and residual.dtype == torch.float32):
            return residual + self._conv4d_gn_relu_hip(x, wq, bq, ws, bs, k, s, p, gn_w, gn_b, eps)[0]
        return self._conv4d_gn_relu_hip(x, wq, bq, ws, bs, k, s, p, gn_w, gn_b, eps, residual=residual)[0]

    def _conv4d_gn_relu_hip(self, x, wq, bq, ws, bs, k, s, p, gn_w, gn_b, eps, keep_pre=False, residual=None):
        x = x.contiguous().float()
        B, Cin, Hq, Wq, Hs, Ws = x.shape
        Cout = wq.shape[0]
        o = lambda n: (n + 2 * p - k) // s + 1
        Hq2, Wq2, Hs2, Ws2 = o(Hq), o(Wq), o(Hs), o(Ws)
        y = torch.empty(B, Cout, Hq2, Wq2, Hs2, Ws2, device=x.device, dtype=torch.float32)
        stats = self._stats(B, Cout, Hq2 * Wq2 * Hs2 * Ws2, x.device)
        f = lambda t: t.detach().contiguous().float()
        wq_, bq_, ws_, bs_, gw, gb = f(wq), f(bq), f(ws), f(bs), f(gn_w), f(gn_b)
        from . import _hip
        nscr = _hip.lib().cpn_conv4d_scratch(B, Cin, Hq, Wq, Hs, Ws, s)
        scr = torch.empty(nscr, dtype=torch.float32, device=x.device) if nscr else None
        scr_p = scr.data_ptr() if scr is not None else 0
        if keep_pre:
            call("cpn_conv4d", x.data_ptr(), wq_.data_ptr(), bq_.data_ptr(), ws_.data_ptr(), bs_.data_ptr(), B, Cin, Cout,
                 Hq, Wq, Hs, Ws, k, s, p, y.data_ptr(), stats.data_ptr(), scr_p, _stream())
            out = torch.empty_like(y)
            call("cpn_gn_relu", y.data_ptr(), stats.data_ptr(), gw.data_ptr(), gb.data_ptr(), 0, float(eps), B, Cout,
                 y[0, 0].numel(), out.data_ptr(), _stream())
            return y, out, stats
        if residual is not None and tuple(residual.shape) != tuple(y.shape):
            raise ValueError("conv4d_gn_relu: residual shape %s != output shape %s" % (tuple(residual.shape), tuple(y.shape)))
        call("cpn_conv4d_gn_relu", x.data_ptr(), wq_.data_ptr(), bq_.data_ptr(), ws_.data_ptr(), bs_.data_ptr(),
             gw.data_ptr(), gb.data_ptr(), 0 if residual is None else residual.data_ptr(), float(eps), B, Cin, Cout, Hq, Wq, Hs, Ws, k, s, p, y.data_ptr(),
             stats.data_ptr(), scr_p, _stream())
        return y, stats

    def correlation_tokens(self, src, trg, fs):
        self._need_gpu(src)
        if _wants_grad(src, trg):
            return _CorrelationFn.apply(self, src.float(), trg.float(), fs)
        return self._correlation(src, trg, fs)[0]

    def _correlation(self, src, trg, fs):
        B, L, C = src.shape
        s_ = src.contiguous().float()
        t_ = trg.contiguous().float()
        out = torch.empty(B, 1, fs, fs, fs, fs, device=src.device, dtype=torch.float32)
        n2 = torch.empty(2, B, L, C, device=src.device, dtype=torch.float32)
        sn, tn = n2[0], n2[1]
        call("cpn_correlation", s_.data_ptr(), t_.data_ptr(), B, L, C, 1e-5, sn.data_ptr(), tn.data_ptr(),
             out.data_ptr(), _stream())
        return out, sn, tn

    def conv_map(self, rgb, w, b, want_nhwc16=False):
        self._need_gpu(rgb)
        if _wants_grad(rgb, w, b):
            return _HipForwardVjp.apply(lambda r, ww, bb: self.conv_map(r, ww, bb)[0], _conv_map_lib,
                                        rgb.float(), w, b), None
        r_, w_, b_ = rgb.contiguous().float(), w.detach().contiguous().float(), b.detach().contiguous().float()
        N, H, W, _ = r_.shape
        out = torch.empty(N, 64, H, W, dtype=torch.float32, device=rgb.device)
        nhwc = torch.empty(N, H, W, 64, dtype=torch.float16, device=rgb.device) if want_nhwc16 else None
        call("cpn_conv_map7x7", r_.data_ptr(), w_.data_ptr(), b_.data_ptr(), N, H, W, out.data_ptr(),
             0 if nhwc is None else nhwc.data_ptr(), _stream())
        return out, nhwc

    def linear_attention(self, q, k, v, channel_major=False, eps=1e-6):
        self._need_gpu(q)
        if _wants_grad(q, k, v):
            return _LinearAttentionFn.apply(self, q.float(), k.float(), v.float(), channel_major, eps)
        q_, k_, v_ = q.contiguous().float(), k.contiguous().float(), v.contiguous().float()
        B, L, H, D = q_.shape
        if D != 32:
            raise ValueError("cpn_linear_attention is built for head dimension 32 (got %d)" % D)
        Dv = v_.shape[2] if channel_major else v_.shape[3]
        nsplit = _linear_attention_splits(L)
        scr = torch.empty(_hip.lib().cpn_linear_attention_scratch(B, H, Dv, nsplit), dtype=torch.float32, device=q.device)
        out = torch.empty_like(v_)
        call("cpn_linear_attention", q_.data_ptr(), k_.data_ptr(), v_.data_ptr(), B, L, H, Dv, int(channel_major), float(eps),
             nsplit, scr.data_ptr(), out.data_ptr(), _stream())
        return out

    def cost_volume_attention(self, q, k, v_corr, fs, residual=None, eps=1e-6):
        self._need_gpu(q)
        B, H, Hs, Ws, Ht, Wt = v_corr.shape
        if _wants_grad(q, k, v_corr) or (residual is not None and _wants_grad(residual)) or Hs != Ws:
            if os.environ.get("CPN_CVA_REFERENCE_ORDER") == "1":
                return cost_volume_attention_reference_order(self, q, k, v_corr, fs, residual, eps)
            return cost_volume_attention_torch(self, q, k, v_corr, fs, residual, eps)
        q_, k_, v_ = q.contiguous().float(), k.contiguous().float(), v_corr.contiguous().float()
        r_ = None if residual is None else residual.contiguous().float()
        P, Dv = Hs * Ws, Ht * Wt
        scr = torch.empty(_hip.lib().cpn_cost_volume_attention_scratch(B, fs * fs, H, P, Dv), dtype=torch.float32, device=q.device)
        out = torch.empty_like(v_)
        call("cpn_cost_volume_attention", q_.data_ptr(), k_.data_ptr(), v_.data_ptr(), 0 if r_ is None else r_.data_ptr(), B, fs,
             H, Hs, Dv, float(eps), scr.data_ptr(), out.data_ptr(), _stream())
        return out

    def resize_bilinear_adjoint(self, x, size):
        return _ResizeAdjointFn.apply(self, x, size)

    def cross_attention(self, c, src_v, trg_v):
        self._need_gpu(c)
        if _wants_grad(c, src_v, trg_v):
            return _CrossAttentionFn.apply(self, c.float(), src_v.float(), trg_v.float())
        c_, s_, t_ = c.contiguous().float(), src_v.contiguous().float(), trg_v.contiguous().float()
        B, H, S, T = c_.shape
        src_attn, trg_attn = torch.empty_like(s_), torch.empty_like(t_)
        call("cpn_cross_attention", c_.data_ptr(), s_.data_ptr(), t_.data_ptr(), B, H, S, T, s_.shape[-1],
             src_attn.data_ptr(), trg_attn.data_ptr(), _stream())
        return src_attn, trg_attn

    def soft_argmax_pair(self, c):
        self._need_gpu(c)
        if _wants_grad(c):
            return _SoftArgmaxPairFn.apply(self, c.contiguous().float())
        return self._soft_argmax_pair_hip(c)

    def _soft_argmax_pair_hip(self, c):
        c = c.contiguous().float()
        B = c.shape[0]
        h = c.shape[-1]
        t_to_s = torch.empty(B, 2, h, h, device=c.device, dtype=torch.float32)
        s_to_t = torch.empty(B, 2, h, h, device=c.device, dtype=torch.float32)
        call("cpn_soft_argmax_pair", c.data_ptr(), B, h, 0.02, t_to_s.data_ptr(), s_to_t.data_ptr(), _stream())
        return t_to_s, s_to_t

    def pose_positional(self, intrinsics, H: int, n: int):
        K = intrinsics.detach().contiguous().float()
        self._need_gpu(K)
        key = (n, str(K.device))
        lin = _LINSPACE.get(key)
        if lin is None:
            lin = _LINSPACE[key] = torch.linspace(-1, 1, steps=n, device=K.device)
        B, V = K.shape[0], K.shape[1]
        out = torch.empty(B, n * n, 6, dtype=torch.float32, device=K.device)
        call("cpn_pose_positional", K.data_ptr(), B, V, float(H), lin.data_ptr(), n, out.data_ptr(), _stream())
        return out

    def pose_tail(self, pose_feat, pose_regressor, rotation_regressor, translation_regressor):
        import ctypes
        x = pose_feat.detach().contiguous().float()
        self._need_gpu(x)
        lin0 = pose_regressor[0]
        nsplit, bias0 = 0, 0
        if x.shape[0] <= 4 and x.shape[1] % 4 == 0 and lin0.weight.is_contiguous() and lin0.weight.shape[0] == 512:
            nsplit = 8
            h = torch.empty(x.shape[0], 512, nsplit, dtype=torch.float32, device=x.device)
            call("cpn_pose_gemv", x.data_ptr(), lin0.weight.data_ptr(), x.shape[0], x.shape[1], 512, nsplit, h.data_ptr(), _stream())
            bias0 = lin0.bias.data_ptr()
        else:
            h = lin0(x).contiguous()
        lins = [pose_regressor[2], pose_regressor[4]] + [m for m in rotation_regressor if isinstance(m, torch.nn.Linear)] + \
               [m for m in translation_regressor if isinstance(m, torch.nn.Linear)]
        shapes = [tuple(m.weight.shape) for m in lins]
        assert shapes == [(256, 512), (256, 256), (64, 128), (32, 64), (6, 32), (64, 128), (32, 64), (3, 32)], shapes
        ptrs = []
        for m in lins:
            for t in (m.weight, m.bias):
                assert t.is_contiguous() and t.dtype == torch.float32 and t.device == h.device
                ptrs.append(t.data_ptr())
        assert len(ptrs) == _hip.POSE_TAIL_TENSORS
        arr = (ctypes.c_void_p * len(ptrs))(*ptrs)
        out = torch.empty(h.shape[0], 4, 4, dtype=torch.float32, device=h.device)
        call("cpn_pose_tail", h.data_ptr(), nsplit, bias0, arr, h.shape[0], out.data_ptr(), _stream())
        return out

    def dual_softmax(self, a):
        self._need_gpu(a)
        return _DualSoftmaxFn.apply(a)

    def corr_mean3(self, corrs):
        if _wants_grad(*corrs):
            return _CorrMean3Fn.apply(self, *(c.float() for c in corrs))
        return self._corr_mean3_hip(corrs)

    def _corr_mean3_hip(self, corrs):
        c0, c1, c2 = (c.detach().contiguous().float() for c in corrs)
        self._need_gpu(c2)
        B, n = c2.shape[0], c2.shape[-1]
        out = torch.empty_like(c2)
        call("cpn_corr_mean3", c0.data_ptr(), c0.shape[-1], c1.data_ptr(), c1.shape[-1], c2.data_ptr(), n, B, out.data_ptr(),
             _stream())
        return out

    def resize_bilinear(self, x, size):
        self._need_gpu(x)
        if _wants_grad(x):
            return _ResizeFn.apply(self, x.float(), size)
        x = x.contiguous().float()
        N, C, h, w = x.shape
        y = torch.empty(N, C, size, size, device=x.device, dtype=torch.float32)
        call("cpn_resize_bilinear_ac", x.data_ptr(), y.data_ptr(), N * C, h, w, size, size, _stream())
        return y
```

### include/coponerf_hip.h

```cpp
#ifndef COPONERF_HIP_H
#define COPONERF_HIP_H

#include <stdint.h>

#ifdef __cplusplus
extern "C" {
#endif

#define CPN_ABI_VERSION 12

#define CPN_E_ARG   (-1)
#define CPN_E_SHAPE (-2)

#define CPN_CAM_STRIDE 96
#define CPN_CAM_TQ    0
#define CPN_CAM_M     16
#define CPN_CAM_AOWN  32
#define CPN_CAM_AOTH  48
#define CPN_CAM_KQ    64
#define CPN_CAM_KC    68
#define CPN_CAM_KO    72
#define CPN_CAM_KN    76


int         cpn_abi_version(void);
const char* cpn_last_error(void);

int cpn_device_cu_count(void);
int cpn_stream_cu_count(void* stream);
int cpn_stream_create_cu_range(int first_cu, int num_cus, void** stream_out);
int cpn_stream_destroy(void* stream);

int cpn_project_rays(const float* cam, const float* uv, long long uv_batch_stride, int B, int V, int R,
                     float* coords9, float* seg, uint8_t* overlaps, void* stream);

int cpn_sample_geometry(const float* cam, const float* coords9, const float* seg, const float* interval,
                        int B, int V, int R, int S, int H, int W,
                        float* pixel_val, float* pt, float* sec_grid, float* pe6, float* loc8, float* lv_u, void* stream);

int cpn_nchw_to_nhwc_f16(const float* src, uint16_t* dst, int N, int C, int h, int w, void* stream);

int cpn_pack_weight_f16(const float* src, int n_out, int k_in, uint16_t* dst, int ld, void* stream);

int cpn_local_hidden(const float* loc8, const float* coords9, const float* w, int ldw, const float* bias,
                     const float* add, int B, int V, int R, int S, int ray0, int nrays, uint16_t* out, void* stream);

#define CPN_TAB_LD    832
#define CPN_NODE_PAD  4
#define CPN_ENC_FRAG_HALVES (13 * 3 * 4 * 64 * 8)
long long cpn_encode_table_nodes(int H, int W);
int cpn_pack_encode_weights(const float* W, int ldw, uint16_t* wfrag, uint16_t* wtab, void* stream);
int cpn_node_features(const uint16_t* map0, const uint16_t* map1, const uint16_t* map2, int H, int W, int nimg,
                      uint16_t* out, void* stream);
int cpn_encode_key(const uint16_t* tab, const uint16_t* map3, int H, int W, const float* pixel_val,
                   const float* sec_grid, const float* pe6, const uint16_t* wfrag, const float* bias,
                   const uint16_t* kwring, const float* kbias, int B, int V, int R, int S, int ray0, int nrays,
                   uint16_t* hid, uint16_t* kh, int kh_units, void* stream);
long long cpn_encode_units(int B, int R, int S, int ray0, int nrays);
int cpn_local_units(int mode, const float* loc8, const float* coords9, const float* w1, int ldw1, const float* b1,
                    const float* add, const uint16_t* w2, int ldw2, const float* b2, const uint16_t* wk2, int ldwk2,
                    const float* bk2, const float* w1b, int ldw1b, const float* b1b, const uint16_t* kh_u, int B, int V,
                    int R, int S, int ray0, int nrays, uint16_t* ce_u, const float* lv_u, float* logits, void* stream);

int cpn_gemm_f16(const uint16_t* A, int lda, const uint16_t* W, int ldw, const float* bias,
                 void* C, int ldc, int M, int N, int K, int relu, int out_f32, void* stream);
int cpn_pack_gemm_frags(const uint16_t* W, int ldw, int N, int K, uint16_t* out, void* stream);
int cpn_gemm_f16_fewrows(const uint16_t* A, int lda, const uint16_t* Wp, const float* bias, float* C, int ldc, int M, int N,
                         int K, int relu, void* stream);

int cpn_attend_hidden(const uint16_t* qa, const uint16_t* qb, const float* logits, const uint16_t* hid, int B, int V,
                      int R, int S, int ray0, int nrays, uint16_t* hbar, float* at_wt, void* stream);

int cpn_attend_units(int mode, const float* loc8, const float* coords9, const float* w1, int ldw1, const float* b1,
                     const float* add, const uint16_t* w2, int ldw2, const float* b2, const uint16_t* wk2, int ldwk2,
                     const float* bk2, const float* w1b, int ldw1b, const float* b1b, const uint16_t* kh_u, const uint16_t* hid,
                     int B, int V, int R, int S, int ray0, int nrays, const float* lv_u, uint16_t* hbar, float* at_wt,
                     float* logits, void* stream);

int cpn_linear_f32(const float* X, int ldx, const float* W, int ldw, const float* bias, const float* res, int ldr,
                   float* Y, int ldy, int M, int N, int K, int relu_in, int relu_out, void* stream);

#define CPN_LIGHTFIELD_PACK_FLOATS (128 * 32 + 128 + 3 * (128 * 416 + 128 + 2 * (128 * 128 + 128)) + 16 * 128 + 16)
int cpn_lightfield_decode(const float* coords9, const float* z_local, const float* wpack, const uint8_t* overlaps,
                          int B, int V, int R, float* rgb, float* valid, float* rgb_raw, void* stream);

#define CPN_RAYC_STRIDE 64
int cpn_ray_outputs(const float* at_wt, const float* pt, const float* uv, long long uv_batch_stride, const float* rayc,
                    const uint8_t* mask2, const float* flow_up, int B, int V, int R, int S, long long* at_wt_max,
                    float* depth_ray, float* t_to_c1, float* t_to_c2, uint8_t* mask_c2, uint8_t* match_mask,
                    float* c2_to_c1, void* stream);


int cpn_node_features_f32(const float* map0, const float* map1, const float* map2, int H, int W, int nimg, float* feat,
                          void* stream);

int cpn_encode_hidden_f32(const float* tab, const float* map3, int H, int W, const float* pixel_val, const float* sec_grid,
                          const float* pe6, const float* w80t, int B, int V, int R, int S, int ray0, int nrays, uint16_t* hs,
                          void* stream);

int cpn_attend_hidden_f32(const float* qa, const float* qb, const uint16_t* hs, int B, int V, int R, int S, int ray0, int nrays,
                          float* hbar, float* at_wt, void* stream);


int cpn_logit_guard(const float* logits, int B, int V, int R, int S, int ray0, int nrays, float* score, int accumulate,
                    void* stream);

int cpn_select_rays(const float* score, int nray, float tau, int* list, int* count, void* stream);

int cpn_encode_hidden_f32_rays(const float* tab, const float* map3, int H, int W, const float* pixel_val, const float* sec_grid,
                               const float* pe6, const float* w80t, int B, int V, int R, int S, const int* rays, int ray0,
                               int nrays, uint16_t* hs, void* stream);
int cpn_attend_hidden_f32_rays(const float* qa, const float* qb, const uint16_t* hs, int B, int V, int R, int S,
                               const int* rays, int ray0, int nrays, float* hbar, float* at_wt, void* stream);


int cpn_attend_hidden_bwd(const uint16_t* qa, const uint16_t* qb, const uint16_t* hid, const float* at_wt,
                          const float* dhbar, const float* dw_ext, int B, int V, int R, int S, int ray0, int nrays,
                          uint16_t* dqa, uint16_t* dqb, uint16_t* dhid, const uint16_t* dqb_acc, void* stream);

int cpn_attend_hidden_bwd_f32(const float* qa, const float* qb, const uint16_t* hs, const float* at_wt, const float* dhbar,
                              const float* dw_ext, int B, int V, int R, int S, int ray0, int nrays, float* dqa, float* dqb,
                              const float* dqb_acc, void* stream);

int cpn_hid_grad_combine(const uint16_t* dkey, const uint16_t* hid, const float* w1, const float* dh1, const float* w2,
                         const float* dh2, int B, int V, int R, int S, int ray0, int nrays, uint16_t* out, void* stream);

int cpn_gemm_f16_combine(const uint16_t* dkh, int lda, const uint16_t* Wt, int ldw, const uint16_t* hid, const float* w1,
                         const float* dh1, const float* w2, const float* dh2, int B, int V, int R, int S, int ray0,
                         int nrays, int K, uint16_t* out, void* stream);

int cpn_gemm_f16_combine_hs(const uint16_t* dkh, int lda, const uint16_t* Wt, int ldw, const uint16_t* hs, const float* w1,
                            const float* dh1, const float* w2, const float* dh2, int B, int V, int R, int S, int ray0,
                            int nrays, int K, uint16_t* out, void* stream);

int cpn_gemm_f16_masked(const uint16_t* A, int lda, const uint16_t* Wt, int ldw, const uint16_t* mask, int ldm, uint16_t* out,
                        int ldc, int M, int N, int K, void* stream);

int cpn_wgrad_skinny_f16(const uint16_t* dY, const uint16_t* X, int ldx, long long M, float* dW, float* db, void* stream);
long long cpn_wgrad_tall_scratch(int N, int K);
int cpn_wgrad_tall_f16(const uint16_t* dY, int ldy, const uint16_t* X, int ldx, long long M, int N, int K, const float* scale,
                       float* part, float* dW, void* stream);
int cpn_local_hidden_bwd(const uint16_t* ds, const uint16_t* out, const float* loc8, const float* coords9,
                         const float* scale, int B, int V, int R, int S, float* dW, float* db, float* dadd, void* stream);

long long cpn_gather_bwd_chunks(int R, int S);
int cpn_gather_rows_bwd_level3(const uint16_t* dxin, int ldx, int col0, int H, int W, const float* pixel_val,
                               const float* sec_grid, int B, int V, int R, int S, int ray0, int nrays, float* dmap3,
                               int32_t* chunk_boxes, void* stream);

long long cpn_scatter_tables_scratch(int H, int W, int B, int V, int R, int S);
int cpn_scale_to_f16(const float* x, long long n, float target, uint32_t* amax_scratch, uint16_t* y, float* scale_out,
                     void* stream);
int cpn_scatter_rows_tables(const uint16_t* d, int ldx, int H, int W, const float* pixel_val, const float* sec_grid, int B,
                            int V, int R, int S, int ray0, int nrays, float* dtab, int32_t* scratch, void* stream);
int cpn_node_features_bwd(const float* dfeat, int H, int W, int nimg, float* dmap0, float* dmap1, float* dmap2,
                          void* stream);
int cpn_gather_tail(const uint16_t* map3, int H, int W, const float* pixel_val, const float* sec_grid, const float* pe6,
                    int B, int V, int R, int S, int ray0, int nrays, uint16_t* xt, void* stream);


long long cpn_conv4d_scratch(int B, int Cin, int Hq, int Wq, int Hs, int Ws, int s);
long long cpn_gn_stats_doubles(int B, int Cout, long long npos);
int cpn_conv4d_gn_relu(const float* x, const float* wq, const float* bq, const float* ws, const float* bs,
                       const float* gn_w, const float* gn_b, const float* residual, float eps, int B, int Cin, int Cout,
                       int Hq, int Wq, int Hs, int Ws, int k, int s, int p, float* y, double* stats, float* scratch,
                       void* stream);

int cpn_conv4d(const float* x, const float* wq, const float* bq, const float* ws, const float* bs, int B, int Cin,
               int Cout, int Hq, int Wq, int Hs, int Ws, int k, int s, int p, float* y, double* stats, float* scratch,
               void* stream);
int cpn_transpose_pairs(const float* x, int N, int P, int Q, float* y, void* stream);

int cpn_conv4d_dgrad(const float* dy, const float* wq, const float* ws, int B, int Cout, int Cin, int Hq, int Wq, int Hs,
                     int Ws, float* dx, void* stream);
int cpn_gn_relu(const float* y, const double* stats, const float* gn_w, const float* gn_b, const float* residual, float eps,
                int B, int C, long long npos, float* out, void* stream);
int cpn_gn_relu_bwd(const float* y, const float* out, const float* dout, const double* stats, const float* gn_w,
                    float eps, int B, int C, long long npos, double* red, float* dy, float* dgn_w, float* dgn_b,
                    void* stream);

long long cpn_conv_wgrad_scratch(int Cin, int Cout);
int cpn_conv_wgrad_planes(const float* x, const float* dy, int B, int Cin, int Cout, int G, int H, int W,
                          float* partial, float* dw, float* db, void* stream);

int cpn_dwconv3x3_wgrad(const float* x, const float* dy, int N, int C, int H, int W, float* dw, float* db,
                        void* stream);

int cpn_dwconv3x3_tokens(const float* x, const float* w, const float* bias, int B, int H, int W, int C, int flip, float* y,
                         void* stream);
long long cpn_dwconv3x3_tokens_wgrad_scratch(int B, int H, int C);
int cpn_dwconv3x3_tokens_wgrad(const float* x, const float* dy, int B, int H, int W, int C, float* partial, float* dw,
                               float* db, void* stream);

int cpn_dual_softmax(const float* a, int B, int L, int M, float* rstat, float* cstat, float* f, void* stream);
int cpn_dual_softmax_bwd(const float* a, const float* rstat, const float* cstat, const float* f, const float* df,
                         int B, int L, int M, float* srow, float* scol, float* da, void* stream);

int cpn_correlation(const float* src, const float* trg, int B, int L, int C, float eps,
                    float* src_n, float* trg_n, float* out, void* stream);
int cpn_l2norm_rows_bwd(const float* x, const float* y, const float* dy, long long rows, int C, float eps,
                        float* dx, void* stream);

long long cpn_wgrad_f32_scratch_floats(long long R, int O, int I);
int cpn_wgrad_f32(const float* dY, int ldy, const float* X, int ldx, long long R, int O, int I, float* dW, float* db,
                  float* scratch, void* stream);

#define CPN_ADAM_SEG_BYTES 48
int cpn_adam_chunk(void);
int cpn_adam_step(const void* segs, const int* blocks, int nblocks, float* exp_avg, float* exp_avg_sq,
                  const float* gscale, const float* gate, const int* counts_in, int* counts_out, double lr,
                  double beta1, double beta2, double eps, void* stream);

int cpn_soft_argmax_pair(const float* c, int B, int h, float beta, float* t_to_s, float* s_to_t, void* stream);
int cpn_soft_argmax_pair_bwd(const float* c, int B, int h, float beta, const float* t_to_s, const float* s_to_t,
                             const float* g_t_to_s, const float* g_s_to_t, float* dc, void* stream);

long long cpn_linear_attention_scratch(int B, int H, int Dv, int nsplit);
int cpn_linear_attention(const float* q, const float* k, const float* v, int B, int L, int H, int Dv,
                         int channel_major, float eps, int nsplit, float* scratch, float* out, void* stream);
long long cpn_linear_attention_bwd_scratch(int B, int L, int H, int Dv, int nsplit);
int cpn_linear_attention_bwd(const float* q, const float* k, const float* v, const float* dout, int B, int L, int H, int Dv,
                             int channel_major, float eps, int nsplit, float* scratch, float* dq, float* dk, float* dv,
                             void* stream);

int cpn_qk_assemble(const float* lin, const float* low, const float* pos, int B, int fs, int h, int w, int nhead, int dim,
                    float* q, float* k, void* stream);

long long cpn_cost_volume_attention_scratch(int B, int L, int H, int P, int Dv);
int cpn_cost_volume_attention(const float* q, const float* k, const float* v_low, const float* residual, int B, int fs,
                              int H, int hs, int Dv, float eps, float* scratch, float* out, void* stream);

long long cpn_conv4d_strided_bwd_scratch(int B, int Cin, int Cout, int Hq, int Wq, int Hs, int Ws, int k, int s, int p);
int cpn_conv4d_strided_bwd(const float* x, const float* dy, const float* wq, const float* ws, int B, int Cin, int Cout,
                           int Hq, int Wq, int Hs, int Ws, int k, int s, int p, float* scratch, float* dx, float* gwq,
                           float* gws, float* gb, void* stream);

int cpn_cross_attention(const float* corr, const float* src_v, const float* trg_v, int B, int H, int S, int T, int C,
                        float* src_attn, float* trg_attn, void* stream);
long long cpn_cross_attention_bwd_scratch(int B, int H, int S, int T);
int cpn_cross_attention_bwd(const float* corr, const float* src_v, const float* trg_v, const float* src_attn,
                            const float* trg_attn, const float* g_src, const float* g_trg, int B, int H, int S, int T, int C,
                            float* scratch, float* dcorr, float* dsrc_v, float* dtrg_v, void* stream);

int cpn_conv_map7x7(const float* rgb, const float* w, const float* bias, int N, int H, int W, float* out_nchw,
                    uint16_t* out_nhwc_f16, void* stream);

int cpn_bn_act(const float* x, const float* res, const float* mean, const float* var, const float* w, const float* b,
               float eps, int N, int C, int HW, int relu, float* y, void* stream);

int cpn_pack_conv_weight(const float* w, int Cout, int Cin, int ksize, float* wp, void* stream);
long long cpn_trunk_conv_scratch_floats(int N, int Hin, int Win, int Cin, int Cout, int ksize, int stride);
int cpn_trunk_conv_bn_act(const float* x, const float* wp, int N, int Hin, int Win, int Cin, int Cout, int ksize, int stride,
                          const float* mean, const float* var, const float* bn_w, const float* bn_b, float eps,
                          const float* res, int relu, float* out_nhwc, float* out_nchw, float* scratch, void* stream);

#define CPN_POSE_TAIL_TENSORS 16
int cpn_pose_positional(const float* intrinsics, int B, int V, float H, const float* lin, int n, float* out, void* stream);
int cpn_pose_gemv(const float* x, const float* W, int B, int K, int O, int nsplit, float* partial, void* stream);
int cpn_pose_tail(const float* h512, int nsplit, const float* bias0, const float* const* weights, int B, float* rel_pose,
                  void* stream);

int cpn_resize_bilinear_ac(const float* src, float* dst, long long planes, int h, int w, int H, int W, void* stream);
int cpn_resize_bilinear_ac_adjoint(const float* g, float* out, long long planes, int h, int w, int H, int W, void* stream);

int cpn_corr_mean3(const float* c0, int h0, const float* c1, int h1, const float* c2, int n, int B, float* out,
                   void* stream);

int cpn_prepare_input(const uint8_t* frames_u8, int B, int Hs, int Ws, int y0, int x0, int H, int W, int R,
                      const int32_t* ray_pix, float* ctx_rgb, float* qry_rgb, void* stream);

int cpn_ssim_warp_blocks(int H, int W);
int cpn_ssim_warp(const float* rgb, const float* flow0, const float* flow1, const uint8_t* mask, const float* window, int B,
                  int H, int W, int h, int w, float* coords, float* maps, float* partial, float* sums, float* loss,
                  float* inv3den, void* stream);
int cpn_ssim_warp_bwd(const float* rgb, const float* coords, const float* maps, const float* window, const float* gout,
                      const float* inv3den, int B, int H, int W, int h, int w, float* gup, float* dflow, void* stream);

int cpn_image_metrics_scratch(int N, int H, int W);
int cpn_image_metrics(const float* pred, const float* target, int N, int H, int W, float* partial, float* out, void* stream);

int cpn_flow_panels(const float* rgb, const float* flow0, const float* flow1, int B, int S, int h, float* warped, uint8_t* mask,
                    uint8_t* overlay, void* stream);
int cpn_depth_jet(const float* depth, long long n, const float* table, float* out, void* stream);
int cpn_attention_entropy_blocks(long long rows);
int cpn_attention_entropy(const float* at_wt, long long rows, int S, int nan_to_zero, float* partial, float* out, void* stream);

#define CPN_LPIPS_LAYERS 5
int cpn_lpips_stem(const float* pred, const float* target, const float* w, const float* bias, int N, int H, int W, float* out,
                   void* stream);
int cpn_lpips_head_scratch(int N, int layers, const int* host_h, const int* host_w);
int cpn_lpips_head(const float* const* host_feat, const float* const* host_lin, const int* host_C, const int* host_h,
                   const int* host_w, int layers, int N, float* partial, float* out, float* per_layer, void* stream);

int cpn_lpips_head_bwd(const float* const* host_feat, const float* const* host_lin, const int* host_C, const int* host_h,
                       const int* host_w, int layers, int N, const float* g, float* const* host_dfeat, void* stream);
int cpn_lpips_stem_bwd(const float* dy, const float* y, const float* pred, const float* w, int N, int H, int W, float* dpred,
                       void* stream);

int cpn_fit_images_u8(const uint8_t* img, int N, int B, int Hi, int Wi, int size, int antialias, float* tmp, float* out,
                      long long batch_stride, long long view_stride, void* stream);
int cpn_camera_path(const float* rel_pose, const double* t, int B, int K, double sway, double turns, float* out, void* stream);
int cpn_pack_frames(const float* rgb, const float* depth, const float* table, int B, int h, int w, uint8_t* out, void* stream);

int cpn_epipolar_lines(const float* intrinsics, const float* rel_pose, const float* gt_rel_pose, const int* points, int B, int P,
                       int W, double* F, double* lines, int* ends, uint8_t* valid, void* stream);
int cpn_epipolar_panels(const float* rgb, const int* points, const float* colors, const int* ends, const uint8_t* valid, int B,
                        int S, int P, int radius, int thickness, float* out, void* stream);
int cpn_mask_contour(const uint8_t* overlay, const uint8_t* mask, int N, int S, uint8_t* out, void* stream);

#define CPN_COMPACT_TILE 1024
#define CPN_COMPACT_FINISH 256
int cpn_depth_points(const float* depth, const float* poses, const float* intrinsics, int K, int B, int S, int y0, int x0, int h,
                     int w, float* xyz, void* stream);
int cpn_depth_votes(const float* depth, const float* poses, const float* intrinsics, int K, int B, int S, int y0, int x0, int h,
                    int w, double px_tol, double rel_tol, uint8_t* votes, float* depth_fused, void* stream);
int cpn_compact_points_scratch(int K, int B, int h, int w);
int cpn_compact_points(const uint8_t* keep, const float* xyz, const float* rgb, int K, int B, int h, int w, int* scratch,
                       float* out_xyz, uint8_t* out_rgb, int* count, void* stream);

int cpn_match_fields(const float* flow0, const float* flow1, const float* intrinsics, const float* rel_pose, int B, int S, int h,
                     float* q, float* cycle, float* epi, uint8_t* inside, void* stream);
int cpn_compact_matches_scratch(int B, int S);
int cpn_compact_matches(const uint8_t* keep, const float* q, const float* cycle, const float* epi, int B, int S, int* scratch,
                        float* xy, float* err, int* count, void* stream);
int cpn_refine_pose(const float* xy, const int* count, const float* intrinsics, const float* rel_pose, int B, int N, int iters,
                    double scale_px, float* pose, double* stats, void* stream);

#define CPN_SPLAT_SCORE_TILE 4096
int cpn_splat_points(const float* xyz, const int* count, const float* poses, const float* intrinsics, int K, int B, int cap, int H,
                     int W, int radius, double near, unsigned long long* zbuf, void* stream);
int cpn_splat_resolve(const unsigned long long* zbuf, const uint8_t* rgb, int K, int B, int cap, int H, int W, int fill,
                      int background, uint8_t* frames, float* depth, int* index, void* stream);
int cpn_splat_score_scratch(int K, int B, int H, int W);
int cpn_splat_score(const uint8_t* frames, const int* index, const uint8_t* target, int K, int B, int H, int W, long long* scratch,
                    long long* stats, void* stream);

int cpn_tsdf_integrate(const float* depth, const uint8_t* valid, const float* rgb, const float* poses, const float* intrinsics,
                       const float* origin, const float* spacing, const float* trunc, int K, int B, int S, int y0, int x0, int h,
                       int w, int Nx, int Ny, int Nz, float* tsdf, uint8_t* weight, float* colour, void* stream);
int cpn_surface_vertices_scratch(int B, int Nx, int Ny, int Nz);
int cpn_surface_vertices(const float* tsdf, const uint8_t* weight, const float* colour, const float* origin, const float* spacing,
                         int B, int Nx, int Ny, int Nz, int min_weight, int capv, int* scratch, float* vert_xyz, uint8_t* vert_rgb,
                         int* nvert, int* cell_vertex, void* stream);
int cpn_surface_faces_scratch(int B, int Nx, int Ny, int Nz);
int cpn_surface_faces(const float* tsdf, const int* cell_vertex, int B, int Nx, int Ny, int Nz, int capf, int* scratch, int* faces,
                      int* nface, void* stream);

#define CPN_RASTER_SMALL 64
#define CPN_RASTER_TILES 256
int cpn_raster_faces(const float* xyz, const int* nvert, const int* faces, const int* nface, const float* poses,
                     const float* intrinsics, int K, int B, int capv, int capf, int H, int W, int cull, double near,
                     unsigned long long* zbuf, void* stream);
int cpn_raster_resolve(const unsigned long long* zbuf, const float* xyz, const uint8_t* rgb, const int* nvert, const int* faces,
                       const float* poses, const float* intrinsics, int K, int B, int capv, int capf, int H, int W, int shade,
                       int background, uint8_t* frames, float* depth, int* index, float* bary, void* stream);

#define CPN_RANSAC_CHUNK 256
int cpn_ransac_hypotheses(const float* xy, const int* count, const float* intrinsics, int B, int N, int Hn, long long seed,
                          double* E, int* sample, uint8_t* valid, void* stream);
int cpn_ransac_score(const double* E, const uint8_t* valid, const float* xy, const int* count, const float* intrinsics,
                     const float* rel_pose, int B, int N, int Hn, double inlier_px, int* partial, void* stream);
int cpn_ransac_finish(const double* E, const uint8_t* valid, const int* partial, const float* xy, const int* count,
                      const float* intrinsics, const float* rel_pose, int B, int N, int Hn, double inlier_px, float* pose,
                      uint8_t* inlier, double* stats, void* stream);

int cpn_ransac_hypotheses5(const float* xy, const int* count, const float* intrinsics, int B, int N, int Hn, long long seed,
                           double* E, int* sample, uint8_t* valid, void* stream);

#ifdef __cplusplus
}
#endif
#endif
```

Measured before the change: 2.914 million rays/s.

## Fold GroupNorm+ReLU of one conv4d into the next conv4d's input loads

Within a conv4d block chain at inference, each layer except the last now skips its separate GroupNorm+ReLU pass and hands its raw output and statistics to the next conv4d. The next conv4d then normalises and applies ReLU to its inputs on load, in both the pooling kernels and the k3s1 scalar and MFMA kernels. This removes one full read/write pass over the 4D correlation tensor per folded layer. The cost is redundant per-element normalisation work inside the conv inner loops, plus extra gamma/beta loads. The render metric may barely depend on this getz trunk path.

```diff
diff --git a/coponerf_amd/csrc/ufc_conv4d.hip b/coponerf_amd/csrc/ufc_conv4d.hip
--- a/coponerf_amd/csrc/ufc_conv4d.hip
+++ b/coponerf_amd/csrc/ufc_conv4d.hip
@@ -57,6 +57,34 @@
     __syncthreads();
     gn_publish(red[0] + red[2] + red[4] + red[6], red[1] + red[3] + red[5] + red[7], stats, b);
 }
+
+__device__ __forceinline__ void gn_mean_rstd(const double* __restrict__ stats, int b, double n, float eps, float& mean,
+                                             float& rstd) {
+    const double m = stats[2 * (size_t)b] / n;
+    const double var = stats[2 * (size_t)b + 1] / n - m * m;
+    mean = (float)m;
+    rstd = (float)(1.0 / sqrt(var + (double)eps));
+}
+
+__device__ __forceinline__ void gn_block_stats(const double* __restrict__ stats, int b, double n, float eps, float& mean,
+                                               float& rstd) {
+    __shared__ float mr[2];
+    if (threadIdx.x == 0) gn_mean_rstd(stats, b, n, eps, mr[0], mr[1]);
+    __syncthreads();
+    mean = mr[0];
+    rstd = mr[1];
+}
+
+__device__ __forceinline__ float gn_relu_value(float v, float mean, float rstd, float gamma, float beta) {
+    return fmaxf(__builtin_fmaf((v - mean) * rstd, gamma, beta), 0.0f);
+}
+
+struct InNorm {
+    const double* stats;
+    const float *gamma, *beta;
+    float eps;
+    double n;
+};
 
 __global__ __launch_bounds__(256) void conv4d_kernel(const float* __restrict__ x, const float* __restrict__ wq,
                                                      const float* __restrict__ bq, const float* __restrict__ ws,
@@ -113,28 +141,49 @@
     gn_publish_block(s1, s2, stats, b);
 }
 
+template <bool NORM>
+struct PoolNorm {
+    long long bc = -1;
+    float mean = 0.f, rstd = 0.f, gamma = 0.f, beta = 0.f;
+    __device__ __forceinline__ void at(const InNorm& in, long long bc_, int Cin) {
+        if (!NORM || bc_ == bc) return;
+        if (bc < 0 || bc_ / Cin != bc / Cin) gn_mean_rstd(in.stats, (int)(bc_ / Cin), in.n, in.eps, mean, rstd);
+        bc = bc_;
+        gamma = in.gamma[bc_ % Cin];
+        beta = in.beta[bc_ % Cin];
+    }
+    __device__ __forceinline__ float operator()(float v) const { return NORM ? gn_relu_value(v, mean, rstd, gamma, beta) : v; }
+};
+
+template <bool NORM>
 __global__ __launch_bounds__(256) void pool_support_kernel(const float* __restrict__ x, int Hs, int Ws, int s, int Os,
-                                                           int Ps_, long long planes, float* __restrict__ out) {
+                                                           int Ps_, long long planes, float* __restrict__ out, InNorm in,
+                                                           int Cin, int HWq) {
     const long long total = planes * Os * Ps_;
+    PoolNorm<NORM> norm;
     for (long long i = (long long)blockIdx.x * blockDim.x + threadIdx.x; i < total; i += (long long)gridDim.x * blockDim.x) {
         const int sx = (int)(i % Ps_);
         long long t = i / Ps_;
         const int sy = (int)(t % Os);
         const long long pl = t / Os;
         const float* base = x + pl * Hs * Ws;
+        norm.at(in, NORM ? pl / HWq : 0, Cin);
         float m = -INFINITY;
         for (int dy = 0; dy < s; ++dy)
             for (int dx = 0; dx < s; ++dx) {
                 const int yy = sy * s + dy, xx = sx * s + dx;
-                if (yy < Hs && xx < Ws) m = fmaxf(m, base[(size_t)yy * Ws + xx]);
+                if (yy < Hs && xx < Ws) m = fmaxf(m, norm(base[(size_t)yy * Ws + xx]));
             }
         out[i] = m;
     }
 }
 
+template <bool NORM>
 __global__ __launch_bounds__(256) void pool_query_kernel(const float* __restrict__ x, int Hq, int Wq, int Hs, int Ws,
-                                                         int s, int Oq, int Pq_, long long bc, float* __restrict__ out) {
+                                                         int s, int Oq, int Pq_, long long bc, float* __restrict__ out,
+                                                         InNorm in, int Cin) {
     const long long P = (long long)Hs * Ws, total = bc * Oq * Pq_ * P;
+    PoolNorm<NORM> norm;
     for (long long i = (long long)blockIdx.x * blockDim.x + threadIdx.x; i < total; i += (long long)gridDim.x * blockDim.x) {
         const long long uv = i % P;
         long long t = i / P;
@@ -142,11 +191,12 @@
         const int qy = (int)(t % Oq);
         const long long c = t / Oq;
         const float* base = x + c * Hq * Wq * P + uv;
+        norm.at(in, c, Cin);
         float m = -INFINITY;
         for (int dy = 0; dy < s; ++dy)
             for (int dx = 0; dx < s; ++dx) {
                 const int yy = qy * s + dy, xx = qx * s + dx;
-                if (yy < Hq && xx < Wq) m = fmaxf(m, base[((size_t)yy * Wq + xx) * P]);
+                if (yy < Hq && xx < Wq) m = fmaxf(m, norm(base[((size_t)yy * Wq + xx) * P]));
             }
         out[i] = m;
     }
@@ -248,14 +298,16 @@
     gn_publish_block(s1, s2, stats, b);
 }
 
-template <int COUT, bool PF, bool DGRAD = false>
+template <int COUT, bool PF, bool DGRAD = false, bool NORM = false>
 __global__ __launch_bounds__(256, PF ? 2 : 4) void conv4d_k3s1_kernel(const float* __restrict__ x, const float* __restrict__ wq,
                                                           const float* __restrict__ bq, const float* __restrict__ ws,
                                                           const float* __restrict__ bs, int Cin, int Hq, int Wq,
                                                           int Hs, int Ws, int cout_total, float* __restrict__ y,
-                                                          double* __restrict__ stats) {
+                                                          double* __restrict__ stats, InNorm in) {
     extern __shared__ __attribute__((aligned(16))) float wl[];
     const int b = blockIdx.z;
+    float in_mean = 0.f, in_rstd = 0.f;
+    if (NORM) gn_block_stats(in.stats, b, in.n, in.eps, in_mean, in_rstd);
     const int o0 = blockIdx.y * COUT;
     for (int i = threadIdx.x; i < Cin * 9 * 2 * COUT; i += 256) {
         const int o = o0 + i % COUT;
@@ -302,7 +354,12 @@
 #pragma unroll
             for (int t = 0; t < 9; ++t) {
                 const f32x4* w4 = reinterpret_cast<const f32x4*>(wl + ((c * 9 + t) * 2) * COUT);
-                const float vq = xv[2 * t], vs = xv[2 * t + 1];
+                float vq = xv[2 * t], vs = xv[2 * t + 1];
+                if (NORM) {
+                    const float ga = in.gamma[c], be = in.beta[c];
+                    vq = off[2 * t] == 0x7ffffff0 ? 0.0f : gn_relu_value(vq, in_mean, in_rstd, ga, be);
+                    vs = off[2 * t + 1] == 0x7ffffff0 ? 0.0f : gn_relu_value(vs, in_mean, in_rstd, ga, be);
+                }
 #pragma unroll
                 for (int o4 = 0; o4 < COUT / 4; ++o4) {
                     const f32x4 a = w4[o4], bb = w4[COUT / 4 + o4];
@@ -344,20 +401,6 @@
     gn_publish_block(s1, s2, stats, b);
 }
 
-__device__ __forceinline__ void gn_block_stats(const double* __restrict__ stats, int b, double n, float eps, float& mean,
-                                               float& rstd) {
-    __shared__ float mr[2];
-    if (threadIdx.x == 0) {
-        const double m = stats[2 * (size_t)b] / n;
-        const double var = stats[2 * (size_t)b + 1] / n - m * m;
-        mr[0] = (float)m;
-        mr[1] = (float)(1.0 / sqrt(var + (double)eps));
-    }
-    __syncthreads();
-    mean = mr[0];
-    rstd = mr[1];
-}
-
 __global__ __launch_bounds__(256) void gn_relu_kernel(const float* y, const double* __restrict__ stats,
                                                       const float* __restrict__ gamma, const float* __restrict__ beta,
                                                       const float* __restrict__ res, float eps, int Cout, long long npos,
@@ -368,18 +411,20 @@
     gn_block_stats(stats, b, (double)Cout * (double)npos, eps, mean, rstd);
     if (pos >= npos) return;
     const size_t idx = ((size_t)b * Cout + o) * npos + pos;
-    const float v = (y[idx] - mean) * rstd * gamma[o] + beta[o];
-    out[idx] = res ? res[idx] + fmaxf(v, 0.0f) : fmaxf(v, 0.0f);
-}
-
-template <int MT, bool DGRAD>
+    const float v = gn_relu_value(y[idx], mean, rstd, gamma[o], beta[o]);
+    out[idx] = res ? res[idx] + v : v;
+}
+
+template <int MT, bool DGRAD, bool NORM = false>
 __global__ __launch_bounds__(256, 2) void conv4d_k3s1_mfma_kernel(const float* __restrict__ x, const float* __restrict__ wq,
                                                                   const float* __restrict__ bq, const float* __restrict__ ws,
                                                                   const float* __restrict__ bs, int Cin, int Hq, int Wq, int Hs,
                                                                   int Ws, int cout_total, float* __restrict__ y,
-                                                                  double* __restrict__ stats) {
+                                                                  double* __restrict__ stats, InNorm in) {
     extern __shared__ __attribute__((aligned(16))) float wl[];
     const int b = blockIdx.z;
+    float in_mean = 0.f, in_rstd = 0.f;
+    if (NORM) gn_block_stats(in.stats, b, in.n, in.eps, in_mean, in_rstd);
     constexpr int CO = MT * 16;
     const int lane = threadIdx.x & 63, wave = threadIdx.x >> 6;
     const int fi = lane & 15, g = lane >> 4;
@@ -419,8 +464,12 @@
 #pragma unroll
             for (int e = 0; e < 4; ++e) acc[mt][e][i] = bias;
         }
-    auto load_group = [&](int c0, f32x4 (&vq)[9], f32x4 (&vs)[3]) {
+    auto load_group = [&](int c0, f32x4 (&vq)[9], f32x4 (&vs)[3], float (&gb)[2]) {
         const int so = c0 * plane;
+        if (NORM) {
+            gb[0] = in.gamma[c0 + g];
+            gb[1] = in.beta[c0 + g];
+        }
 #pragma unroll
         for (int k = 0; k < 9; ++k) vq[k] = __builtin_bit_cast(f32x4, __builtin_amdgcn_raw_buffer_load_b128(rs, offq[k], so, 0));
 #pragma unroll
@@ -436,7 +485,19 @@
             for (int e = 0; e < 4; ++e) acc[mt][e] = __builtin_amdgcn_mfma_f32_16x16x4f32(a, v[e], acc[mt][e], 0, 0, 0);
         }
     };
-    auto compute_group = [&](int c0, const f32x4 (&vq)[9], const f32x4 (&vs)[3]) {
+    auto normalise = [&](f32x4 v, int off, float ga, float be) {
+        if (off == kOOB) return f32x4{0.f, 0.f, 0.f, 0.f};
+#pragma unroll
+        for (int e = 0; e < 4; ++e) v[e] = gn_relu_value(v[e], in_mean, in_rstd, ga, be);
+        return v;
+    };
+    auto compute_group = [&](int c0, f32x4 (&vq)[9], f32x4 (&vs)[3], const float (&gb)[2]) {
+        if (NORM) {
+#pragma unroll
+            for (int k = 0; k < 9; ++k) vq[k] = normalise(vq[k], offq[k], gb[0], gb[1]);
+#pragma unroll
+            for (int k = 0; k < 3; ++k) vs[k] = normalise(vs[k], offs[k], gb[0], gb[1]);
+        }
 #pragma unroll
         for (int i = 0; i < 3; ++i) {
             const f32x4 r = vs[i];
@@ -457,7 +518,8 @@
         __builtin_amdgcn_sched_barrier(0);
     };
     f32x4 q0[9], s0[3], q1[9], s1v[3];
-    load_group(0, q0, s0);
+    float gb0[2] = {0.f, 0.f}, gb1[2] = {0.f, 0.f};
+    load_group(0, q0, s0, gb0);
     if (cout_total < CO)
         for (int i = threadIdx.x; i < 18 * Cin * CO; i += 256)
             if (i % CO >= cout_total) wl[i] = 0.0f;
@@ -483,11 +545,11 @@
     }
     __syncthreads();
     for (int c0 = 0; c0 < Cin; c0 += 8) {
-        if (c0 + 4 < Cin) load_group(c0 + 4, q1, s1v);
-        compute_group(c0, q0, s0);
+        if (c0 + 4 < Cin) load_group(c0 + 4, q1, s1v, gb1);
+        compute_group(c0, q0, s0, gb0);
         if (c0 + 4 < Cin) {
-            if (c0 + 8 < Cin) load_group(c0 + 8, q0, s0);
-            compute_group(c0 + 4, q1, s1v);
+            if (c0 + 8 < Cin) load_group(c0 + 8, q0, s0, gb0);
+            compute_group(c0 + 4, q1, s1v, gb1);
         }
     }
     double s1 = 0.0, s2 = 0.0;
@@ -625,61 +687,51 @@
            ((uintptr_t)y % 16) == 0;
 }
 
-template <bool DGRAD>
+template <bool DGRAD, bool NORM = false>
 void launch_conv4d_mfma(hipStream_t st, const float* x, const float* wq, const float* bq, const float* ws, const float* bs, int B,
-                        int cred, int cprod, int Hq, int Wq, int Hs, int Ws, float* y, double* stats) {
+                        int cred, int cprod, int Hq, int Wq, int Hs, int Ws, float* y, double* stats, const InNorm& in = InNorm{}) {
     const dim3 g2(cpn_cdiv((long long)Hq * Wq * Hs * Ws, 256), 1, B);
-    auto* kernel = cprod <= 16 ? conv4d_k3s1_mfma_kernel<1, DGRAD> : conv4d_k3s1_mfma_kernel<2, DGRAD>;
+    auto* kernel = cprod <= 16 ? conv4d_k3s1_mfma_kernel<1, DGRAD, NORM> : conv4d_k3s1_mfma_kernel<2, DGRAD, NORM>;
     hipLaunchKernelGGL(kernel, g2, dim3(256), conv4d_mfma_lds(cred, cprod), st, x, wq, bq, ws, bs, cred, Hq, Wq, Hs, Ws, cprod, y,
-                       stats);
-}
-
-}
-
-extern "C" long long cpn_gn_stats_doubles(int B, int Cout, long long npos) {
-    const long long wg = std::max<long long>((long long)cpn_cdiv(npos, 256) * Cout, (long long)cpn_cdiv(npos, 64));
-    return 3LL * B + 2LL * B * wg;
-}
-
-extern "C" long long cpn_conv4d_scratch(int B, int Cin, int Hq, int Wq, int Hs, int Ws, int s) {
-    if (s <= 1) return 0;
-    const SGeo g{B, Cin, 0, Hq, Wq, Hs, Ws, 0, s, 0, pooled_size(Hq, s), pooled_size(Wq, s), pooled_size(Hs, s), pooled_size(Ws, s)};
-    return g.n_ps() + g.n_pq();
-}
-
-extern "C" int cpn_conv4d(const float* x, const float* wq, const float* bq, const float* ws, const float* bs, int B,
-                          int Cin, int Cout, int Hq, int Wq, int Hs, int Ws, int k, int s, int p, float* y,
-                          double* stats, float* scratch, void* stream) {
-    CPN_REQUIRE(x && wq && bq && ws && bs && y && stats, CPN_E_ARG, "cpn_conv4d: null pointer");
+                       stats, in);
+}
+
+template <bool NORM>
+int conv4d_launch(const char* who, const InNorm& in, const float* x, const float* wq, const float* bq, const float* ws,
+                  const float* bs, int B, int Cin, int Cout, int Hq, int Wq, int Hs, int Ws, int k, int s, int p, float* y,
+                  double* stats, float* scratch, void* stream) {
+    CPN_REQUIRE(x && wq && bq && ws && bs && y && stats, CPN_E_ARG, "%s: null pointer", who);
     CPN_REQUIRE(B > 0 && B < 65536 && Cin > 0 && Cout > 0 && Cout < 65536 && k > 0 && s > 0 && p >= 0, CPN_E_SHAPE,
-                "cpn_conv4d: bad shape");
+                "%s: bad shape", who);
     SGeo g;
     CPN_REQUIRE(make_geo(B, Cin, Cout, Hq, Wq, Hs, Ws, k, s, p, &g), CPN_E_SHAPE,
-                "cpn_conv4d: conv output (%d) and pooled size (%d) of the two branches disagree", g.Oq, pooled_size(Hq, s));
+                "%s: conv output (%d) and pooled size (%d) of the two branches disagree", who, g.Oq, pooled_size(Hq, s));
     const int Oq = g.Oq, Pq_ = g.Pq, Os = g.Os, Ps_ = g.Ps;
     const long long npos = g.npos();
     const hipStream_t st = (hipStream_t)stream;
     dim3 grid(cpn_cdiv(npos, 256), Cout, B);
     const size_t wbytes = (size_t)Cin * 9 * 2 * Cout * sizeof(float);
     if (k == 3 && s == 1 && p == 1 && conv4d_mfma_ok(Cin, Cout, Ws, npos, x, y)) {
-        launch_conv4d_mfma<false>(st, x, wq, bq, ws, bs, B, Cin, Cout, Hq, Wq, Hs, Ws, y, stats);
+        launch_conv4d_mfma<false, NORM>(st, x, wq, bq, ws, bs, B, Cin, Cout, Hq, Wq, Hs, Ws, y, stats, in);
     } else if (k == 3 && s == 1 && p == 1 && (Cout == 8 || Cout == 32) && wbytes <= 64 * 1024 &&
         (long long)Cin * npos * 4 < 0x7ffffff0LL) {
         const bool small = (long long)B * npos <= 131072;
         const int per = (Cout == 8 && small) ? 4 : 8;
         dim3 g1(cpn_cdiv(npos, 256), Cout / per, B);
         const size_t wb = wbytes / (Cout / per);
-        auto* kernel = per == 4 ? conv4d_k3s1_kernel<4, true> : small ? conv4d_k3s1_kernel<8, true> : conv4d_k3s1_kernel<8, false>;
-        hipLaunchKernelGGL(kernel, g1, dim3(256), wb, st, x, wq, bq, ws, bs, Cin, Hq, Wq, Hs, Ws, Cout, y, stats);
+        auto* kernel = per == 4 ? conv4d_k3s1_kernel<4, true, false, NORM>
+                       : small  ? conv4d_k3s1_kernel<8, true, false, NORM>
+                                : conv4d_k3s1_kernel<8, false, false, NORM>;
+        hipLaunchKernelGGL(kernel, g1, dim3(256), wb, st, x, wq, bq, ws, bs, Cin, Hq, Wq, Hs, Ws, Cout, y, stats, in);
     } else if (s > 1 && scratch) {
         float* psv = scratch;
         float* pqv = scratch + (size_t)B * Cin * Hq * Wq * Os * Ps_;
         const long long planes = (long long)B * Cin * Hq * Wq;
         const long long n1 = planes * Os * Ps_, n2 = (long long)B * Cin * Oq * Pq_ * Hs * Ws;
-        hipLaunchKernelGGL(pool_support_kernel, dim3((unsigned)std::min<long long>(cpn_cdiv(n1, 256), 65536)), dim3(256), 0,
-                           st, x, Hs, Ws, s, Os, Ps_, planes, psv);
-        hipLaunchKernelGGL(pool_query_kernel, dim3((unsigned)std::min<long long>(cpn_cdiv(n2, 256), 65536)), dim3(256), 0,
-                           st, x, Hq, Wq, Hs, Ws, s, Oq, Pq_, (long long)B * Cin, pqv);
+        hipLaunchKernelGGL(pool_support_kernel<NORM>, dim3((unsigned)std::min<long long>(cpn_cdiv(n1, 256), 65536)), dim3(256), 0,
+                           st, x, Hs, Ws, s, Os, Ps_, planes, psv, in, Cin, Hq * Wq);
+        hipLaunchKernelGGL(pool_query_kernel<NORM>, dim3((unsigned)std::min<long long>(cpn_cdiv(n2, 256), 65536)), dim3(256), 0,
+                           st, x, Hq, Wq, Hs, Ws, s, Oq, Pq_, (long long)B * Cin, pqv, in, Cin);
         if (Cout == 8 && (size_t)Cin * k * k * 16 * sizeof(float) <= 48 * 1024)
             hipLaunchKernelGGL(conv4d_pooled_c8_kernel, dim3(cpn_cdiv(npos, 256), 1, B), dim3(256),
                                (size_t)Cin * k * k * 16 * sizeof(float), st, psv, pqv, wq, bq, ws, bs, Cin, Hq, Wq, Hs, Ws, k, s, p,
@@ -688,11 +740,55 @@
             hipLaunchKernelGGL(conv4d_pooled_kernel, grid, dim3(256), 0, st, psv, pqv, wq, bq, ws, bs, Cin, Hq, Wq, Hs, Ws, k, s,
                                p, Oq, Pq_, Os, Ps_, y, stats);
     } else {
+        CPN_REQUIRE(!NORM, CPN_E_SHAPE, "%s: no kernel for k=%d s=%d p=%d Cin=%d Cout=%d (k3 s1 p1 fast forms, or stride > 1 with scratch)",
+                    who, k, s, p, Cin, Cout);
         hipLaunchKernelGGL(conv4d_kernel, grid, dim3(256), 0, st, x, wq, bq, ws, bs, Cin, Hq, Wq, Hs, Ws, k, s, p, Oq,
                            Pq_, Os, Ps_, y, stats);
     }
-    CPN_LAUNCH_CHECK("cpn_conv4d");
+    CPN_LAUNCH_CHECK(who);
     return 0;
+}
+
+inline InNorm make_in_norm(const double* in_stats, const float* in_gn_w, const float* in_gn_b, float in_eps, int Cin, int Hq, int Wq,
+                           int Hs, int Ws) {
+    return InNorm{in_stats, in_gn_w, in_gn_b, in_eps, (double)Cin * ((double)Hq * Wq * Hs * Ws)};
+}
+
+}
+
+extern "C" long long cpn_gn_stats_doubles(int B, int Cout, long long npos) {
+    const long long wg = std::max<long long>((long long)cpn_cdiv(npos, 256) * Cout, (long long)cpn_cdiv(npos, 64));
+    return 3LL * B + 2LL * B * wg;
+}
+
+extern "C" long long cpn_conv4d_scratch(int B, int Cin, int Hq, int Wq, int Hs, int Ws, int s) {
+    if (s <= 1) return 0;
+    const SGeo g{B, Cin, 0, Hq, Wq, Hs, Ws, 0, s, 0, pooled_size(Hq, s), pooled_size(Wq, s), pooled_size(Hs, s), pooled_size(Ws, s)};
+    return g.n_ps() + g.n_pq();
+}
+
+extern "C" int cpn_conv4d(const float* x, const float* wq, const float* bq, const float* ws, const float* bs, int B,
+                          int Cin, int Cout, int Hq, int Wq, int Hs, int Ws, int k, int s, int p, float* y,
+                          double* stats, float* scratch, void* stream) {
+    return conv4d_launch<false>("cpn_conv4d", InNorm{}, x, wq, bq, ws, bs, B, Cin, Cout, Hq, Wq, Hs, Ws, k, s, p, y, stats, scratch,
+                                stream);
+}
+
+extern "C" int cpn_conv4d_folded_ok(int Cin, int Cout, int Hq, int Wq, int Hs, int Ws, int k, int s, int p) {
+    if (Cin <= 0 || Cout <= 0 || k <= 0 || s <= 0 || p < 0) return 0;
+    if (s > 1) return 1;
+    const long long npos = (long long)Hq * Wq * Hs * Ws;
+    return k == 3 && p == 1 && (Cout == 8 || Cout == 32) && (size_t)Cin * 9 * 2 * Cout * sizeof(float) <= 64 * 1024 &&
+           (long long)Cin * npos * 4 < 0x7ffffff0LL;
+}
+
+extern "C" int cpn_conv4d_folded(const float* x, const double* in_stats, const float* in_gn_w, const float* in_gn_b, float in_eps,
+                                 const float* wq, const float* bq, const float* ws, const float* bs, int B, int Cin, int Cout,
+                                 int Hq, int Wq, int Hs, int Ws, int k, int s, int p, float* y, double* stats, float* scratch,
+                                 void* stream) {
+    CPN_REQUIRE(in_stats && in_gn_w && in_gn_b, CPN_E_ARG, "cpn_conv4d_folded: null pointer");
+    return conv4d_launch<true>("cpn_conv4d_folded", make_in_norm(in_stats, in_gn_w, in_gn_b, in_eps, Cin, Hq, Wq, Hs, Ws), x, wq, bq,
+                               ws, bs, B, Cin, Cout, Hq, Wq, Hs, Ws, k, s, p, y, stats, scratch, stream);
 }
 
 extern "C" int cpn_conv4d_dgrad(const float* dy, const float* wq, const float* ws, int B, int Cout, int Cin, int Hq, int Wq,
@@ -714,7 +810,7 @@
     dim3 g1(cpn_cdiv(npos, 256), Cin / per, B);
     auto* kernel = per == 4 ? conv4d_k3s1_kernel<4, false, true> : conv4d_k3s1_kernel<8, false, true>;
     hipLaunchKernelGGL(kernel, g1, dim3(256), wb, (hipStream_t)stream, dy, wq, (const float*)nullptr, ws, (const float*)nullptr,
-                       Cout, Hq, Wq, Hs, Ws, Cin, dx, (double*)nullptr);
+                       Cout, Hq, Wq, Hs, Ws, Cin, dx, (double*)nullptr, InNorm{});
     CPN_LAUNCH_CHECK("cpn_conv4d_dgrad");
     return 0;
 }
@@ -746,6 +842,20 @@
                                   void* stream) {
     CPN_REQUIRE(gn_w && gn_b, CPN_E_ARG, "cpn_conv4d_gn_relu: null pointer");
     int rc = cpn_conv4d(x, wq, bq, ws, bs, B, Cin, Cout, Hq, Wq, Hs, Ws, k, s, p, y, stats, scratch, stream);
+    if (rc) return rc;
+    SGeo g;
+    make_geo(B, Cin, Cout, Hq, Wq, Hs, Ws, k, s, p, &g);
+    return cpn_gn_relu(y, stats, gn_w, gn_b, residual, eps, B, Cout, g.npos(), y, stream);
+}
+
+extern "C" int cpn_conv4d_gn_relu_folded(const float* x, const double* in_stats, const float* in_gn_w, const float* in_gn_b,
+                                         float in_eps, const float* wq, const float* bq, const float* ws, const float* bs,
+                                         const float* gn_w, const float* gn_b, const float* residual, float eps, int B, int Cin,
+                                         int Cout, int Hq, int Wq, int Hs, int Ws, int k, int s, int p, float* y, double* stats,
+                                         float* scratch, void* stream) {
+    CPN_REQUIRE(gn_w && gn_b, CPN_E_ARG, "cpn_conv4d_gn_relu_folded: null pointer");
+    int rc = cpn_conv4d_folded(x, in_stats, in_gn_w, in_gn_b, in_eps, wq, bq, ws, bs, B, Cin, Cout, Hq, Wq, Hs, Ws, k, s, p, y, stats,
+                               scratch, stream);
     if (rc) return rc;
     SGeo g;
     make_geo(B, Cin, Cout, Hq, Wq, Hs, Ws, k, s, p, &g);
diff --git a/coponerf_amd/getz.py b/coponerf_amd/getz.py
--- a/coponerf_amd/getz.py
+++ b/coponerf_amd/getz.py
@@ -247,11 +247,20 @@
 
     def forward(self, x, ops, residual=None):
         last = len(self.conv4d) - 1
+        defer = getattr(ops, "conv4d_deferred", None) if FOLD_PASSES and not torch.is_grad_enabled() else None
+        pre = None
         for i, blk in enumerate(self.conv4d):
             c4, gn = blk[0], blk[1]
             args = (x, c4.query_conv.weight, c4.query_conv.bias, c4.supp_conv.weight, c4.supp_conv.bias, c4.k, c4.s, c4.p,
                     gn.weight, gn.bias, gn.eps)
-            x = ops.conv4d_gn_relu(*args, residual=residual) if (i == last and residual is not None) else ops.conv4d_gn_relu(*args)
+            kw = {} if pre is None else {"pre": pre}
+            if i == last and residual is not None:
+                kw["residual"] = residual
+            pre = None
+            if defer is not None and i < last and not kw:
+                nx = self.conv4d[i + 1][0]
+                pre = defer(*args, (nx.query_conv.out_channels, nx.k, nx.s, nx.p))
+            x = None if pre is not None else ops.conv4d_gn_relu(*args, **kw)
         return x
 
 
@@ -275,6 +284,7 @@
 BATCH_VIEWS = os.environ.get("CPN_GETZ_BATCH_VIEWS", "1") != "0"
 FUSED_TRUNK = os.environ.get("CPN_GETZ_FUSED_TRUNK", "1") != "0"
 HIP_TRUNK_TAIL = os.environ.get("CPN_GETZ_HIP_TRUNK_TAIL", "1") != "0"
+FOLD_PASSES = os.environ.get("CPN_GETZ_FOLD", "1") != "0"
 FUSED_POSE_ENDS = os.environ.get("CPN_GETZ_FUSED_POSE_ENDS", "1") != "0"
 HIP_TRUNK_MAX_POSITIONS = int(os.environ.get("CPN_GETZ_HIP_TRUNK_MAX_POSITIONS", "2048"))
 CORR_MEAN3_TRAIN = os.environ.get("CPN_CORR_MEAN3_TRAIN", "1") != "0"
diff --git a/coponerf_amd/ufc_ops.py b/coponerf_amd/ufc_ops.py
--- a/coponerf_amd/ufc_ops.py
+++ b/coponerf_amd/ufc_ops.py
@@ -1,6 +1,7 @@
 from __future__ import annotations
 
 import os
+from collections import namedtuple
 
 import torch
 import torch.nn.functional as F
@@ -8,6 +9,8 @@
 
 from . import _hip
 from ._hip import call
+
+PreNorm = namedtuple("PreNorm", "y stats gn_w gn_b eps")
 
 
 def _stream() -> int:
@@ -566,7 +569,22 @@
         pool[1] = i + ((n + 1) // 2) * 2
         return pool[0][i:i + n]
 
-    def conv4d_gn_relu(self, x, wq, bq, ws, bs, k, s, p, gn_w, gn_b, eps, residual=None):
+    def conv4d_deferred(self, x, wq, bq, ws, bs, k, s, p, gn_w, gn_b, eps, nxt):
+        self._need_gpu(x)
+        if _wants_grad(x, wq, bq, ws, bs, gn_w, gn_b):
+            return None
+        Hq, Wq, Hs, Ws = ((n + 2 * p - k) // s + 1 for n in x.shape[2:])
+        if not _hip.lib().cpn_conv4d_folded_ok(wq.shape[0], nxt[0], Hq, Wq, Hs, Ws, nxt[1], nxt[2], nxt[3]):
+            return None
+        return self._conv4d_gn_relu_hip(x, wq, bq, ws, bs, k, s, p, gn_w, gn_b, eps, defer=True)
+
+    def conv4d_gn_relu(self, x, wq, bq, ws, bs, k, s, p, gn_w, gn_b, eps, residual=None, pre=None):
+        if pre is not None:
+            if _wants_grad(wq, bq, ws, bs, gn_w, gn_b) or (residual is not None and _wants_grad(residual)):
+                raise RuntimeError("conv4d_gn_relu: a deferred normalisation is an inference form (no gradients)")
+            if residual is not None and not (residual.is_contiguous() and residual.dtype == torch.float32):
+                return residual + self._conv4d_gn_relu_hip(None, wq, bq, ws, bs, k, s, p, gn_w, gn_b, eps, pre=pre)[0]
+            return self._conv4d_gn_relu_hip(None, wq, bq, ws, bs, k, s, p, gn_w, gn_b, eps, residual=residual, pre=pre)[0]
         self._need_gpu(x)
         if _wants_grad(x, wq, bq, ws, bs, gn_w, gn_b) or (residual is not None and _wants_grad(residual)):
             y = _Conv4dGnReluFn.apply(self, x.float(), wq, bq, ws, bs, gn_w, gn_b, k, s, p, eps)
@@ -575,8 +593,9 @@
             return residual + self._conv4d_gn_relu_hip(x, wq, bq, ws, bs, k, s, p, gn_w, gn_b, eps)[0]
         return self._conv4d_gn_relu_hip(x, wq, bq, ws, bs, k, s, p, gn_w, gn_b, eps, residual=residual)[0]
 
-    def _conv4d_gn_relu_hip(self, x, wq, bq, ws, bs, k, s, p, gn_w, gn_b, eps, keep_pre=False, residual=None):
-        x = x.contiguous().float()
+    def _conv4d_gn_relu_hip(self, x, wq, bq, ws, bs, k, s, p, gn_w, gn_b, eps, keep_pre=False, residual=None, defer=False,
+                            pre=None):
+        x = pre.y if pre is not None else x.contiguous().float()
         B, Cin, Hq, Wq, Hs, Ws = x.shape
         Cout = wq.shape[0]
         o = lambda n: (n + 2 * p - k) // s + 1
@@ -598,8 +617,18 @@
             return y, out, stats
         if residual is not None and tuple(residual.shape) != tuple(y.shape):
             raise ValueError("conv4d_gn_relu: residual shape %s != output shape %s" % (tuple(residual.shape), tuple(y.shape)))
+        res_p = 0 if residual is None else residual.data_ptr()
+        if defer:
+            call("cpn_conv4d", x.data_ptr(), wq_.data_ptr(), bq_.data_ptr(), ws_.data_ptr(), bs_.data_ptr(), B, Cin, Cout,
+                 Hq, Wq, Hs, Ws, k, s, p, y.data_ptr(), stats.data_ptr(), scr_p, _stream())
+            return PreNorm(y, stats, gw, gb, float(eps))
+        if pre is not None:
+            call("cpn_conv4d_gn_relu_folded", x.data_ptr(), pre.stats.data_ptr(), pre.gn_w.data_ptr(), pre.gn_b.data_ptr(),
+                 pre.eps, wq_.data_ptr(), bq_.data_ptr(), ws_.data_ptr(), bs_.data_ptr(), gw.data_ptr(), gb.data_ptr(), res_p,
+                 float(eps), B, Cin, Cout, Hq, Wq, Hs, Ws, k, s, p, y.data_ptr(), stats.data_ptr(), scr_p, _stream())
+            return y, stats
         call("cpn_conv4d_gn_relu", x.data_ptr(), wq_.data_ptr(), bq_.data_ptr(), ws_.data_ptr(), bs_.data_ptr(),
-             gw.data_ptr(), gb.data_ptr(), 0 if residual is None else residual.data_ptr(), float(eps), B, Cin, Cout, Hq, Wq, Hs, Ws, k, s, p, y.data_ptr(),
+             gw.data_ptr(), gb.data_ptr(), res_p, float(eps), B, Cin, Cout, Hq, Wq, Hs, Ws, k, s, p, y.data_ptr(),
              stats.data_ptr(), scr_p, _stream())
         return y, stats
 
diff --git a/include/coponerf_hip.h b/include/coponerf_hip.h
--- a/include/coponerf_hip.h
+++ b/include/coponerf_hip.h
@@ -169,6 +169,15 @@
 int cpn_conv4d(const float* x, const float* wq, const float* bq, const float* ws, const float* bs, int B, int Cin,
                int Cout, int Hq, int Wq, int Hs, int Ws, int k, int s, int p, float* y, double* stats, float* scratch,
                void* stream);
+int cpn_conv4d_folded_ok(int Cin, int Cout, int Hq, int Wq, int Hs, int Ws, int k, int s, int p);
+int cpn_conv4d_folded(const float* x, const double* in_stats, const float* in_gn_w, const float* in_gn_b, float in_eps,
+                      const float* wq, const float* bq, const float* ws, const float* bs, int B, int Cin, int Cout, int Hq,
+                      int Wq, int Hs, int Ws, int k, int s, int p, float* y, double* stats, float* scratch, void* stream);
+int cpn_conv4d_gn_relu_folded(const float* x, const double* in_stats, const float* in_gn_w, const float* in_gn_b,
+                              float in_eps, const float* wq, const float* bq, const float* ws, const float* bs,
+                              const float* gn_w, const float* gn_b, const float* residual, float eps, int B, int Cin,
+                              int Cout, int Hq, int Wq, int Hs, int Ws, int k, int s, int p, float* y, double* stats,
+                              float* scratch, void* stream);
 int cpn_transpose_pairs(const float* x, int N, int P, int Q, float* y, void* stream);
 
 int cpn_conv4d_dgrad(const float* dy, const float* wq, const float* ws, int B, int Cout, int Cin, int Hq, int Wq, int Hs,
```

Result: slower. 2.861 million rays/s (-1.8%).
